# polli-labs/linnaeus

Measured on AMD Instinct MI355X. Metric: images/sec (train fwd+bwd) mFormerV1_sm 3x224x224, higher is better.
Workload: dtype bf16; 1 GPU; mFormerV1_sm train step (forward + 4-task CE loss + backward + AdamW (one HIP launch)), bf16 operands / fp32 accumulate+residual, batch 256/GPU, 3x224x224 synthetic, DropPath 0.2, gradient checkpointing off; per_gpu_batch=256, global_batch=256, parallelism=dp1, grad_mode=direct

## Files before the change

### include/lnx.h

```cpp
#ifndef LNX_H
#define LNX_H
#include <stdint.h>

#ifdef __cplusplus
extern "C" {
#endif

#define LNX_F32 0
#define LNX_BF16 1

const char* lnx_last_error(void);
int lnx_version(void);
int lnx_device_cus(void);
int lnx_set_cu_margin(int cus);
int lnx_set_deterministic(int on);
int lnx_get_deterministic(void);
int lnx_tile_sched_static(void);

typedef struct lnx_rowmap {
    int group, pad, off;
} lnx_rowmap;

enum { LNX_ACT_NONE = 0, LNX_ACT_GELU = 1, LNX_ACT_RELU = 2, LNX_ACT_GELU_BWD = 3, LNX_ACT_RELU_BWD = 4,
       LNX_ACT_GELU_D = 5, LNX_ACT_MUL_AUX = 6 };
// ... 201 lines not shown
int lnx_dwconv7_wgrad_kept(const lnx_dwconv_wgrad_args* args, const int* perm, const int* nkeep, void* stream);
int64_t lnx_dwconv7_wgrad_ws_floats(int B, int H, int W, int C, int x_dtype, int dy_dtype);

enum { LNX_ROPE_COS = 0, LNX_ROPE_ROTATE = 1 };
int lnx_rope_cos_table(const float* freqs , int heads, int H, int W, float* cos_out ,
                       float* dsin_out ,
                       void* stream);
int lnx_rope_cos_table_hd(const float* freqs, int heads, int head_dim, int H, int W, float* cos_out, float* dsin_out, void* stream);
int lnx_rope_cossin_table_hd(const float* freqs, int heads, int head_dim, int H, int W, float* cos_out, float* sin_out, float* dsin_out, void* stream);
#define LNX_ROPE_TABLES_MAX 24
typedef struct {
    const float* freqs;
    float* cos_out;
    float* dsin_out;
    int heads, H, W;
    int head_dim;
    int rope_mode;
    float* sin_out;
} lnx_rope_table;
int lnx_rope_cos_tables(const lnx_rope_table* tables, int n, void* stream);
int64_t lnx_attn_bwd_ws_floats(int B, int N, int heads);
int64_t lnx_attn_bwd_ws_floats_hd(int B, int N, int heads, int head_dim);

typedef struct lnx_attn_args {
    int dtype;
    int B, N, E, heads;
    const void* qkv;
    const float* cos_tab;
    void* o;
    float* lse;
    const unsigned char* drop_mask;
    float drop_inv_keep;
    int head_dim;
    int rope_mode;
    const float* sin_tab;
} lnx_attn_args;
int lnx_attn_fwd(const lnx_attn_args* args, void* stream);

typedef struct lnx_attn_bwd_args {
    int dtype;
    int B, N, E, heads;
    const void* qkv;
    const float* cos_tab;
    const void* o;
    const float* lse;
    const void* d_o;
    void* dqkv;
    float* freq_ws;
    float* delta;
    const unsigned char* drop_mask;
    float drop_inv_keep;
    const float* dsin_tab;
    float* dfreqs;
    int defer_freqs;
    int head_dim;
    int rope_mode;
    const float* sin_tab;
    int grid_w;
} lnx_attn_bwd_args;
#define LNX_ATTN_DEFER_MAX 16
int lnx_attn_bwd_flush(void* stream);
int lnx_attn_bwd_discard(void);
int lnx_attn_bwd(const lnx_attn_bwd_args* args, void* stream);
int lnx_attn_bwd_sized(const lnx_attn_bwd_args* args, int64_t freq_ws_floats, void* stream);
int lnx_attn_fwd_compact(const lnx_attn_args* args, const int* nkeep, void* stream);
int lnx_attn_bwd_compact(const lnx_attn_bwd_args* args, const int* nkeep, int64_t freq_ws_floats, void* stream);

enum { LNX_ATTN_KERNEL_NONE = 0, LNX_ATTN_KERNEL_RES4 = 1 , LNX_ATTN_KERNEL_RES8 = 2 ,
       LNX_ATTN_KERNEL_TILED4 = 3 , LNX_ATTN_KERNEL_TILED8 = 4  };
int lnx_attn_dispatch(int dtype, int N, int head_dim, int has_drop_mask);
int lnx_last_attn_kernel(void);
int lnx_last_attn_bwd_launches(void);

int lnx_im2col_stem(const float* x, int B, int Cin, int H, int W, void* patches, int dtype, int ldp, void* stream);

typedef struct lnx_stem_args {
    const float* x;
    const void* w;
    const float* bias;
    const float* ln_w;
    const float* ln_b;
    void* patches;
    void* pre;
    float* y;
    float* mean;
    float* rstd;
    int B, Cin, H, W, Cout;
    float eps;
} lnx_stem_args;
int lnx_stem_fwd_ok(int dtype, int Cin, int H, int W, int Cout);
int lnx_stem_fwd(const lnx_stem_args* args, void* stream);

int lnx_scale_cast(const float* in, int64_t ldin, lnx_rowmap in_map, const float* rowscale, int rows_per_sample, void* out,
                   int out_dtype, int64_t ldout, int M, int C, void* stream);

#define LNX_DROP_LIST_INTS(B) (2 * (B) + 2)
#define LNX_DROP_PARTITION_MAX 64
int lnx_drop_partition(const float* scales, int n_calls, int B, const unsigned char* call_mask, const int* rows_per_sample, int* lists, void* stream);
int lnx_scale_cast_compact(const float* in, int64_t ldin, const float* rowscale, int rows_per_sample, const int* perm, const int* m_dev, void* out,
                           int out_dtype, int64_t ldout, int M, int C, void* stream);

int lnx_copy_dropped_rows(const float* src, float* dst, int64_t ld, const int* perm, const int* nkeep, int B, int rows_per_sample, int C, void* stream);

int lnx_set_drop_compact(int on);
int64_t lnx_drop_compact_branches(void);
int64_t lnx_drop_compact_conv_blocks(void);
int lnx_set_last_cls(int on);
int64_t lnx_last_cls_blocks(void);

int lnx_layerscale_bwd(const float* g, const void* z, int dtype, const float* gamma, const float* rowscale,
                       int rows_per_sample, void* dz, float* dgamma, int M, int C, void* stream);

int lnx_layerscale_apply_wgrad(const float* s, const float* t, int64_t lds, const float* w, const float* b, int64_t ldw, const float* gamma, float* dw, float* db,
                               int64_t lddw, float* dgamma, int C, int K, void* stream);

int lnx_dropout_mul(void* x, int dtype, const unsigned char* mask, float inv_keep, int M, int C, void* stream);
int lnx_dropout_residual(const void* z, int z_dtype, const unsigned char* mask, float inv_keep, const float* rowscale, int rows_per_sample,
                         const float* res, float* out, int M, int C, void* stream);

int lnx_fill_rows(const float* vec, float* out, int64_t ldout, lnx_rowmap map, int M, int C, void* stream);
int lnx_layerscale_bwd_ws(const float* g, const void* z, int dtype, const float* gamma, const float* rowscale, int rows_per_sample, void* dz,
                          float* dgamma, int M, int C, float* ws, int64_t ws_floats, void* stream);
int64_t lnx_layerscale_bwd_ws_floats(int M, int C);
int lnx_colsum_rows(const float* in, int64_t ldin, lnx_rowmap map, float* out, int M, int C, void* stream);

int lnx_agg2_fwd(const float* a, const float* b, const float* w2, const float* bias1, float* out, int M, int C, void* stream);
int lnx_agg2_bwd(const float* dout, const float* a, const float* b, const float* w2, float* da, float* db_, float* dw2,
                 float* dbias1, int M, int C, void* stream);

int lnx_pack_meta(const float* meta, int width, int off, int dim, void* out, int dtype, int B, void* stream);

typedef struct lnx_meta_head_args {
    int B, C;
    int dim, off;
    const float* meta;
    int meta_width;
    float eps;
    const float* w0;
    int ldw0;
    const float *b0, *ln0_w, *ln0_b;
    const float* w1;
    int ldw1;
    const float *b1, *ln1_w, *ln1_b;
    const float* w2;
    int ldw2;
    const float *b2, *ln2_w, *ln2_b;
    float* t0;
    float *h0, *x, *h1, *n1, *h2;
    float *m0, *r0, *m1, *r1, *m2, *r2;
    float* tok;
    int64_t tok_row_stride, tok_row_offset;
// ... 604 lines not shown
```

### linnaeus_amd/_lib.py

```python
from __future__ import annotations

import ctypes as C
import os

_HERE = os.path.dirname(os.path.abspath(__file__))
LIB_PATH = os.environ.get("LNX_LIB_PATH") or os.path.join(_HERE, "liblnx_hip.so")

F32, BF16 = 0, 1
ACT_NONE, ACT_GELU, ACT_RELU, ACT_GELU_BWD, ACT_RELU_BWD, ACT_GELU_D, ACT_MUL_AUX = 0, 1, 2, 3, 4, 5, 6
TN_WS_FLOATS = 256 * (256 * 128 + 256)
DROP_PARTITION_MAX = 64


def drop_list_ints(B: int) -> int:
    return 2 * B + 2
ADDR_PLAIN, ADDR_PATCH2 = 0, 1


class LnxError(RuntimeError):
    pass


class RowMap(C.Structure):
    _fields_ = [("group", C.c_int), ("pad", C.c_int), ("off", C.c_int)]
# ... 320 lines not shown
        if hasattr(_lib, "lnx_hier_refine_fwd"):
            _lib.lnx_hier_refine_fwd.argtypes = [C.POINTER(HierRefineArgs), C.c_void_p]
            _lib.lnx_hier_refine_bwd.argtypes = [C.POINTER(HierRefineArgs), C.c_void_p]
            _lib.lnx_hier_refine_launches.restype = C.c_int64
        if hasattr(_lib, "lnx_abstain_act"):
            _lib.lnx_abstain_act.argtypes = [C.POINTER(AbstainActArgs), C.c_void_p]
            _lib.lnx_ppo_advantages.argtypes = [C.POINTER(PpoAdvArgs), C.c_void_p]
            _lib.lnx_ppo_loss_fwd.argtypes = [C.POINTER(PpoLossArgs), C.c_void_p]
            _lib.lnx_ppo_loss_bwd.argtypes = [C.POINTER(PpoLossArgs), C.c_void_p, C.c_void_p]
            _lib.lnx_abstain_launches.restype = C.c_int64
        if hasattr(_lib, "lnx_preprocess"):
            _lib.lnx_resize_taps.argtypes = [C.c_int, C.c_int, C.c_int]
            _lib.lnx_resize_coeffs.argtypes = [C.c_int, C.c_int, C.c_int, C.c_void_p, C.c_void_p]
            _lib.lnx_preprocess_scratch_bytes.argtypes = [C.POINTER(PreprocessImage), C.c_int, C.c_int, C.c_int, C.c_int]
            _lib.lnx_preprocess_scratch_bytes.restype = C.c_int64
            _lib.lnx_preprocess.argtypes = [C.POINTER(PreprocessArgs), C.c_void_p]
            _lib.lnx_preprocess.restype = C.c_int
        if hasattr(_lib, "lnx_meta_mask"):
            _lib.lnx_meta_mask.argtypes = [C.POINTER(MetaMaskArgs), C.c_void_p]
            _lib.lnx_meta_mask.restype = C.c_int
        if hasattr(_lib, "lnx_drop_partition"):
            _lib.lnx_drop_partition.argtypes = [C.c_void_p, C.c_int, C.c_int, C.c_char_p, C.POINTER(C.c_int), C.c_void_p, C.c_void_p]
            _lib.lnx_copy_dropped_rows.argtypes = [C.c_void_p, C.c_void_p, C.c_int64, C.c_void_p, C.c_void_p, C.c_int, C.c_int, C.c_int, C.c_void_p]
            _lib.lnx_drop_compact_branches.restype = C.c_int64
            if hasattr(_lib, "lnx_drop_compact_conv_blocks"):
                _lib.lnx_drop_compact_conv_blocks.restype = C.c_int64
                _lib.lnx_dwconv7_fwd_kept.argtypes = [C.POINTER(DwconvArgs), C.c_void_p, C.c_void_p, C.c_void_p]
                _lib.lnx_dwconv7_wgrad_kept.argtypes = [C.POINTER(DwconvWgradArgs), C.c_void_p, C.c_void_p, C.c_void_p]
            _lib.lnx_scale_cast_compact.argtypes = [C.c_void_p, C.c_int64, C.c_void_p, C.c_int, C.c_void_p, C.c_void_p, C.c_void_p, C.c_int, C.c_int64, C.c_int, C.c_int,
                                                    C.c_void_p]
        if hasattr(_lib, "lnx_last_cls_blocks"):
            _lib.lnx_set_last_cls.argtypes = [C.c_int]
            _lib.lnx_last_cls_blocks.restype = C.c_int64
        if hasattr(_lib, "lnx_plan_forward_tail"):
            _lib.lnx_plan_forward_tail.argtypes = [C.c_void_p, C.c_void_p, C.c_void_p, C.c_void_p, C.c_void_p]
            _lib.lnx_plan_trunk_valid.argtypes = [C.c_void_p]
        if hasattr(_lib, "lnx_plan_set_trainable"):
            _lib.lnx_plan_unit_name.argtypes = [C.c_void_p, C.c_int]
            _lib.lnx_plan_unit_name.restype = C.c_char_p
            _lib.lnx_plan_set_trainable.argtypes = [C.c_void_p, C.c_char_p]
        if hasattr(_lib, "lnx_gemm_tn_query"):
            _lib.lnx_gemm_tn_query.argtypes = [C.POINTER(WgradArgs), C.POINTER(TnLaunch)]
        if hasattr(_lib, "lnx_layernorm_fwd_query"):
            _lib.lnx_layernorm_fwd_query.argtypes = [C.POINTER(LnArgs), C.POINTER(LnLaunch)]
            _lib.lnx_layernorm_bwd_query.argtypes = [C.POINTER(LnBwdArgs), C.POINTER(LnLaunch)]
        older = bool(os.environ.get("LNX_LIB_PATH")) and os.environ.get("LNX_LIB_OLDER") == "1"
        for name in EXPORTS:
            if not hasattr(_lib, name) and not older:
                raise LnxError(f"{LIB_PATH} does not export {name}; rebuild it")
    return _lib


def set_deterministic(on: bool) -> bool:
    return bool(lib().lnx_set_deterministic(1 if on else 0))


def is_deterministic() -> bool:
    return bool(lib().lnx_get_deterministic())


def check(rc: int, what: str) -> None:
    if rc != 0:
        raise LnxError(f"{what} failed (rc={rc}): {lib().lnx_last_error().decode()}")


AUG_CLAMP, AUG_POSTERIZE, AUG_SOLARIZE, AUG_SOLARIZE_ADD, AUG_INVERT, AUG_BRIGHTNESS, AUG_CONTRAST = range(7)

NT_KERNEL_NONE, NT_KERNEL_V1, NT_KERNEL_V2, NT_KERNEL_SKINNY, NT_KERNEL_V4, NT_KERNEL_FP8, NT_KERNEL_V7, NT_KERNEL_MX8, NT_KERNEL_V9, NT_KERNEL_EXPERIMENT = 0, 1, 2, 3, 4, 6, 7, 8, 9, 15

ROPE_COS, ROPE_ROTATE = 0, 1

ATTN_KERNEL_NONE, ATTN_KERNEL_RES4, ATTN_KERNEL_RES8, ATTN_KERNEL_TILED4, ATTN_KERNEL_TILED8 = range(5)

EXPORTS = [
    "lnx_last_error", "lnx_version", "lnx_device_cus", "lnx_set_cu_margin", "lnx_set_deterministic", "lnx_get_deterministic", "lnx_tile_sched_static",
    "lnx_gemm_nt", "lnx_last_nt_kernel", "lnx_nt_kernel_launches", "lnx_nt_dispatch", "lnx_gemm_tn", "lnx_gemm_tn_query", "lnx_gemm_tn_flush", "lnx_gemm_tn_discard", "lnx_amax", "lnx_quantize_fp8", "lnx_gemm_nt_fp8", "lnx_quantize_mxfp8", "lnx_gemm_nt_mxfp8", "lnx_dropout_mul", "lnx_dropout_residual", "lnx_plan_dropout_bytes", "lnx_plan_set_dropout", "lnx_plan_attn_dropout_bytes", "lnx_plan_set_attn_dropout",
    "lnx_layernorm_fwd", "lnx_layernorm_bwd", "lnx_layernorm_bwd_flush", "lnx_layernorm_bwd_discard", "lnx_layernorm_fwd_query", "lnx_layernorm_bwd_query",
    "lnx_dwconv7_fwd", "lnx_dwconv7_fwd_kept", "lnx_dwconv7_wgrad", "lnx_dwconv7_wgrad_kept", "lnx_dwconv7_wgrad_ws_floats",
    "lnx_gemm_nt_group_ok", "lnx_gemm_nt_group", "lnx_rope_cos_table", "lnx_rope_cos_table_hd", "lnx_rope_cossin_table_hd", "lnx_rope_cos_tables", "lnx_attn_bwd_ws_floats", "lnx_attn_bwd_ws_floats_hd", "lnx_attn_fwd", "lnx_attn_bwd", "lnx_attn_bwd_sized", "lnx_attn_fwd_compact", "lnx_attn_bwd_compact", "lnx_attn_bwd_flush", "lnx_attn_bwd_discard", "lnx_attn_dispatch", "lnx_last_attn_kernel", "lnx_last_attn_bwd_launches",
    "lnx_im2col_stem", "lnx_scale_cast", "lnx_scale_cast_compact", "lnx_drop_partition", "lnx_copy_dropped_rows", "lnx_set_drop_compact", "lnx_drop_compact_branches", "lnx_drop_compact_conv_blocks", "lnx_set_last_cls", "lnx_last_cls_blocks", "lnx_layerscale_bwd", "lnx_layerscale_bwd_ws", "lnx_layerscale_bwd_ws_floats", "lnx_layerscale_apply_wgrad", "lnx_fill_rows", "lnx_colsum_rows",
    "lnx_agg2_fwd", "lnx_agg2_bwd", "lnx_pack_meta", "lnx_meta_heads_supported", "lnx_meta_heads_fwd", "lnx_meta_heads_bwd", "lnx_meta_heads_bwd_part_floats", "lnx_prep_weights", "lnx_prep_blocks", "lnx_softce", "lnx_softce_multi", "lnx_taxonomy_rows", "lnx_stem_fwd", "lnx_stem_fwd_ok", "lnx_adamw_blocks", "lnx_grad_sumsq", "lnx_adamw_step", "lnx_ademamix_step", "lnx_sgd_step", "lnx_optim_launches", "lnx_grad_sumsq_guarded", "lnx_adamw_step_guarded", "lnx_ademamix_step_guarded", "lnx_sgd_step_guarded", "lnx_muon_layout", "lnx_muon_step", "lnx_muon_launches", "lnx_muon_partition", "lnx_muon_orthogonalize", "lnx_muon_apply_packed", "lnx_gradnorm_sumsq", "lnx_gradnorm_update",
    "lnx_metrics_table_sizes", "lnx_metrics_update", "lnx_predict", "lnx_resize_taps", "lnx_resize_coeffs", "lnx_preprocess_scratch_bytes", "lnx_preprocess", "lnx_hier_loss_fwd", "lnx_hier_loss_bwd",
    "lnx_hier_refine_fwd", "lnx_hier_refine_bwd", "lnx_hier_refine_launches",
    "lnx_abstain_act", "lnx_ppo_advantages", "lnx_ppo_loss_fwd", "lnx_ppo_loss_bwd", "lnx_abstain_launches",
    "lnx_mix_rows", "lnx_mix_meta", "lnx_meta_mask",
    "lnx_aug_pointwise", "lnx_aug_saturation", "lnx_aug_rowstat", "lnx_aug_rescale", "lnx_aug_affine", "lnx_aug_stencil", "lnx_erase_rects", "lnx_u8hwc_to_f32chw",
    "lnx_convmlp_supported", "lnx_convmlp_fwd", "lnx_convmlp_bwd", "lnx_convmlp_bwd_ws_floats",
    "lnx_plan_create", "lnx_plan_destroy", "lnx_plan_workspace_bytes", "lnx_plan_num_params", "lnx_plan_param_name",
    "lnx_plan_param_numel", "lnx_plan_num_drop_calls", "lnx_plan_logits_numel", "lnx_plan_logits_offset", "lnx_plan_logits_ld",
    "lnx_plan_bind", "lnx_plan_forward", "lnx_plan_forward_tail", "lnx_plan_trunk_valid", "lnx_plan_backward", "lnx_plan_backward_into", "lnx_plan_segment_params", "lnx_plan_profile_begin", "lnx_plan_profile_end", "lnx_plan_profile_begin_spans", "lnx_plan_profile_end_ex", "lnx_plan_set_wgrad_stream", "lnx_plan_set_meta_stream",
    "lnx_plan_num_units", "lnx_plan_unit_name", "lnx_plan_param_unit", "lnx_plan_set_trainable", "lnx_plan_first_trained_unit", "lnx_plan_last_backward_units",
]


class MetaHeadArgs(C.Structure):
    _fields_ = [
        ("B", C.c_int), ("C", C.c_int), ("dim", C.c_int), ("off", C.c_int),
        ("meta", C.c_void_p), ("meta_width", C.c_int), ("eps", C.c_float),
        ("w0", C.c_void_p), ("ldw0", C.c_int), ("b0", C.c_void_p), ("ln0_w", C.c_void_p), ("ln0_b", C.c_void_p),
        ("w1", C.c_void_p), ("ldw1", C.c_int), ("b1", C.c_void_p), ("ln1_w", C.c_void_p), ("ln1_b", C.c_void_p),
        ("w2", C.c_void_p), ("ldw2", C.c_int), ("b2", C.c_void_p), ("ln2_w", C.c_void_p), ("ln2_b", C.c_void_p),
        ("t0", C.c_void_p), ("h0", C.c_void_p), ("x", C.c_void_p), ("h1", C.c_void_p), ("n1", C.c_void_p), ("h2", C.c_void_p),
        ("m0", C.c_void_p), ("r0", C.c_void_p), ("m1", C.c_void_p), ("r1", C.c_void_p), ("m2", C.c_void_p), ("r2", C.c_void_p),
        ("tok", C.c_void_p), ("tok_row_stride", C.c_int64), ("tok_row_offset", C.c_int64),
    ]


class MetaHeadBwdArgs(C.Structure):
    _fields_ = [
        ("B", C.c_int), ("C", C.c_int), ("dim", C.c_int),
        ("g", C.c_void_p), ("g_row_stride", C.c_int64), ("g_row_offset", C.c_int64),
        ("w1t", C.c_void_p), ("ldw1t", C.c_int), ("w2t", C.c_void_p), ("ldw2t", C.c_int),
        ("ln0_w", C.c_void_p), ("ln1_w", C.c_void_p), ("ln2_w", C.c_void_p),
# ... 42 lines not shown
class LnLaunch(C.Structure):
    _fields_ = [("G", C.c_int), ("V", C.c_int), ("pair", C.c_int), ("full", C.c_int), ("mx", C.c_int), ("grid", C.c_int), ("cols", C.c_int), ("slices", C.c_int)]


class RopeTable(C.Structure):
    _fields_ = [
        ("freqs", C.c_void_p), ("cos_out", C.c_void_p), ("dsin_out", C.c_void_p),
        ("heads", C.c_int), ("H", C.c_int), ("W", C.c_int), ("head_dim", C.c_int),
        ("rope_mode", C.c_int), ("sin_out", C.c_void_p),
    ]


class DwconvArgs(C.Structure):
    _fields_ = [
        ("B", C.c_int), ("H", C.c_int), ("W", C.c_int), ("C", C.c_int),
        ("x", C.c_void_p), ("x_dtype", C.c_int), ("w49", C.c_void_p), ("bias", C.c_void_p),
        ("flip", C.c_int), ("res", C.c_void_p), ("y", C.c_void_p), ("y_dtype", C.c_int),
    ]


class DwconvWgradArgs(C.Structure):
    _fields_ = [
        ("B", C.c_int), ("H", C.c_int), ("W", C.c_int), ("C", C.c_int),
        ("x", C.c_void_p), ("x_dtype", C.c_int), ("dy", C.c_void_p), ("dy_dtype", C.c_int),
        ("dw", C.c_void_p), ("db", C.c_void_p),
        ("ws", C.c_void_p), ("ws_floats", C.c_int64),
    ]


class AttnArgs(C.Structure):
    _fields_ = [
        ("dtype", C.c_int), ("B", C.c_int), ("N", C.c_int), ("E", C.c_int), ("heads", C.c_int),
        ("qkv", C.c_void_p), ("cos_tab", C.c_void_p), ("o", C.c_void_p), ("lse", C.c_void_p),
        ("drop_mask", C.c_void_p), ("drop_inv_keep", C.c_float), ("head_dim", C.c_int),
        ("rope_mode", C.c_int), ("sin_tab", C.c_void_p),
    ]


class AttnBwdArgs(C.Structure):
    _fields_ = [
        ("dtype", C.c_int), ("B", C.c_int), ("N", C.c_int), ("E", C.c_int), ("heads", C.c_int),
        ("qkv", C.c_void_p), ("cos_tab", C.c_void_p), ("o", C.c_void_p), ("lse", C.c_void_p),
        ("d_o", C.c_void_p), ("dqkv", C.c_void_p), ("freq_ws", C.c_void_p), ("delta", C.c_void_p),
        ("drop_mask", C.c_void_p), ("drop_inv_keep", C.c_float),
        ("dsin_tab", C.c_void_p), ("dfreqs", C.c_void_p), ("defer_freqs", C.c_int), ("head_dim", C.c_int),
        ("rope_mode", C.c_int), ("sin_tab", C.c_void_p), ("grid_w", C.c_int),
    ]


class PrepDesc(C.Structure):
    _fields_ = [
        ("src", C.c_void_p), ("dst", C.c_void_p), ("dst_t", C.c_void_p),
        ("rows", C.c_int), ("cols", C.c_int), ("ld", C.c_int), ("ld_t", C.c_int),
        ("P", C.c_int), ("mode", C.c_int), ("block_start", C.c_int),
    ]


PREP_CAST, PREP_CONV_PERM, PREP_DW49 = 0, 1, 2


class ConvMlpArgs(C.Structure):
    _fields_ = [
        ("dtype", C.c_int), ("M", C.c_int), ("C", C.c_int),
        ("ln", C.c_void_p), ("w1", C.c_void_p), ("b1", C.c_void_p), ("w2", C.c_void_p), ("b2", C.c_void_p),
        ("gamma", C.c_void_p), ("rowscale", C.c_void_p), ("rows_per_sample", C.c_int),
        ("x", C.c_void_p), ("out", C.c_void_p), ("z", C.c_void_p),
        ("y", C.c_void_p), ("ln_w", C.c_void_p), ("ln_b", C.c_void_p), ("ln_eps", C.c_float), ("ln_out", C.c_void_p),
        ("mean", C.c_void_p), ("rstd", C.c_void_p),
        ("perm", C.c_void_p), ("m_dev", C.c_void_p),
    ]


class ConvMlpBwdArgs(C.Structure):
    _fields_ = [
        ("dtype", C.c_int), ("M", C.c_int), ("C", C.c_int),
        ("g", C.c_void_p), ("ln", C.c_void_p), ("z", C.c_void_p), ("w1", C.c_void_p), ("b1", C.c_void_p),
        ("w2t", C.c_void_p), ("w1t", C.c_void_p), ("gamma", C.c_void_p), ("rowscale", C.c_void_p), ("rows_per_sample", C.c_int),
        ("act", C.c_void_p), ("dh", C.c_void_p), ("dz", C.c_void_p), ("dln", C.c_void_p), ("dgamma", C.c_void_p),
# ... 33 lines not shown
```

### linnaeus_amd/csrc/api.cpp

```cpp
#include <hip/hip_runtime.h>
#include <stdarg.h>
#include <stdio.h>
#include <stdlib.h>
#include <string.h>

#include <atomic>
#include <mutex>

#include "../../include/lnx.h"

static thread_local char g_err[1024] = "";

void lnx_set_error(const char* fmt, ...) {
    va_list ap;
    va_start(ap, fmt);
    vsnprintf(g_err, sizeof(g_err), fmt, ap);
    va_end(ap);
}

extern "C" const char* lnx_last_error(void) { return g_err; }
extern "C" int lnx_version(void) { return 120; }
extern "C" int lnx_device_cus(void) {
    int dev = 0;
    if (hipGetDevice(&dev) != hipSuccess) return -1;
    hipDeviceProp_t prop;
    if (hipGetDeviceProperties(&prop, dev) != hipSuccess) return -1;
    return prop.multiProcessorCount;
}

static std::atomic<int> g_cu_margin{-1};
int persistent_cus(int cus) {
    int m = g_cu_margin.load(std::memory_order_relaxed);
    if (m < 0) {
        const char* e = getenv("LNX_CU_MARGIN");
        m = e ? atoi(e) : 0;
        if (m < 0) m = 0;
        g_cu_margin.store(m, std::memory_order_relaxed);
    }
    const int room = cus - m;
    return room < 8 ? 8 : room;
}
void set_cu_margin(int m) { g_cu_margin.store(m < 0 ? 0 : m, std::memory_order_relaxed); }
static std::atomic<int> g_deterministic{-1};
bool deterministic() {
    int d = g_deterministic.load(std::memory_order_relaxed);
    if (d < 0) {
        const char* e = getenv("LNX_DETERMINISTIC");
        d = e && atoi(e) == 1 ? 1 : 0;
        int unset = -1;
        if (!g_deterministic.compare_exchange_strong(unset, d, std::memory_order_relaxed)) d = unset;
    }
    return d != 0;
}
extern "C" int lnx_get_deterministic(void) { return deterministic() ? 1 : 0; }
// ... 42 lines not shown
```

### linnaeus_amd/csrc/attention.hip

```cpp
#include <stdlib.h>

#include <atomic>
#include <vector>

#include "common.hpp"
#include "../../include/lnx.h"

namespace {

constexpr int BT = 64;

typedef __attribute__((ext_vector_type(4))) short s16x4_t;

template <typename T, int HD = 64> struct AT {
    static_assert(HD == 32 || HD == 64 || HD == 128, "head_dim 32, 64 or 128");
    static constexpr int EPV = TT<T>::EPV;
    static constexpr int NKK = HD * (int)sizeof(T) / 64;
    static constexpr int ND = HD / 16;
    static constexpr int ROWB = HD * sizeof(T);
    static constexpr int NCH = ROWB / 16;
    static constexpr int SWZ = (NCH < 8 ? NCH : 8) - 1;
    static constexpr int TRB = ROWB + (sizeof(T) == 2 ? 32 : 16);
    static constexpr int ROW_IMG = BT * ROWB;
    static constexpr int TR_IMG = BT * TRB;
// ... 305 lines not shown
    static __device__ __forceinline__ float prep(float m) {
        if constexpr (sizeof(T) == 2) return m * L2E;
        else return m;
    }
    static __device__ __forceinline__ float sub(float x, float mp) {
        if constexpr (sizeof(T) == 2) return __builtin_amdgcn_exp2f(fmaf(x, L2E, -mp));
        else return expf(x - mp);
    }
    static __device__ __forceinline__ float clamped(float x, float mp) {
        if constexpr (sizeof(T) == 2) return __builtin_amdgcn_exp2f(fminf(fmaf(x, L2E, -mp), 0.f));
        else return expf(fminf(x - mp, 0.f));
    }
};

struct AttnP {
    const void* qkv;
    const float* cos_tab;
    void* o;
    float* lse;
    const void* d_o;
    void* dqkv;
    float* fpart;
    const float* dsin;
    float* delta;
    int B, N, E, heads;
    int qtiles;
    const unsigned char* amask = nullptr;
    float a_inv_keep = 1.0f;
    int Np = 0;
    const float* sin_tab = nullptr;
    int W = 1;
    float* fwave = nullptr;
    const int* nkeep = nullptr;
};

template <int HD = 64> __device__ __forceinline__ float* freq_wave_slot(const AttnP& p) {
    if (p.fwave == nullptr) return nullptr;
    const int wave = __builtin_amdgcn_readfirstlane(threadIdx.x >> 6), lane = threadIdx.x & 63;
    float* fw = p.fwave + ((int64_t)blockIdx.x * FREQ_WAVES + wave) * HD;
    if ((lane & 15) == 0) {
#pragma unroll
        for (int dt = 0; dt < HD / 16; ++dt)
#pragma unroll
            for (int pr = 0; pr < 2; ++pr) {
                const int j = 8 * dt + 2 * (lane >> 4) + pr;
                fw[j] = 0.f;
                fw[HD / 2 + j] = 0.f;
            }
    }
    return fw;
}

template <typename T, int HD = 64, bool ROT = false>
__device__ __forceinline__ void dkv_epilogue(const AttnP& p, const f32x4_t (&dk)[HD / 16], const f32x4_t (&dv)[HD / 16], const T* __restrict__ kb, int64_t ld, int C,
                                             int b, int head, int key, int s, int g, float* fl, float* fw) {
    const int kc = min(key, p.N - 1);
    const T* kraw = kb + (int64_t)kc * ld;
    const float* cpr = p.cos_tab + ((int64_t)max(kc - p.E, 0) * p.heads + head) * (HD / 2);
    const float* sxp = p.dsin + ((int64_t)max(kc - p.E, 0) * p.heads + head) * (HD / 2);
    const float* syp = sxp + (int64_t)(p.N - p.E) * p.heads * (HD / 2);
    constexpr int ND = HD / 16;
    float kr[ND][4], cr[ND][2], gp[ND][2], dx[ND][2], dy[ND][2];
    float sr[ROT ? ND : 1][2];
    const bool rope = p.E < p.N;
#pragma unroll
    for (int dt = 0; dt < ND; ++dt) {
// ... 34 lines not shown
        float ok[ND][4];
#pragma unroll
        for (int dt = 0; dt < ND; ++dt) {
            const float c0 = img ? cr[dt][0] : 1.0f, c1 = img ? cr[dt][1] : 1.0f;
            if constexpr (ROT) {
                const float s0 = img ? sr[dt][0] : 0.f, s1 = img ? sr[dt][1] : 0.f;
                ok[dt][0] = dk[dt][0] * c0 + dk[dt][1] * s0; ok[dt][1] = dk[dt][1] * c0 - dk[dt][0] * s0;
                ok[dt][2] = dk[dt][2] * c1 + dk[dt][3] * s1; ok[dt][3] = dk[dt][3] * c1 - dk[dt][2] * s1;
                const float x0 = kr[dt][0] * c0 - kr[dt][1] * s0, x1 = kr[dt][0] * s0 + kr[dt][1] * c0;
                const float x2 = kr[dt][2] * c1 - kr[dt][3] * s1, x3 = kr[dt][2] * s1 + kr[dt][3] * c1;
                gp[dt][0] = img ? dk[dt][1] * x0 - dk[dt][0] * x1 : 0.f;
                gp[dt][1] = img ? dk[dt][3] * x2 - dk[dt][2] * x3 : 0.f;
                continue;
            }
            ok[dt][0] = dk[dt][0] * c0; ok[dt][1] = dk[dt][1] * c0; ok[dt][2] = dk[dt][2] * c1; ok[dt][3] = dk[dt][3] * c1;
            gp[dt][0] = img ? dk[dt][0] * kr[dt][0] + dk[dt][1] * kr[dt][1] : 0.f;
            gp[dt][1] = img ? dk[dt][2] * kr[dt][2] + dk[dt][3] * kr[dt][3] : 0.f;
        }
        store_row<T, HD>(dkp, ok, g, row);
    }
    {
        float ov[ND][4];
#pragma unroll
        for (int dt = 0; dt < ND; ++dt)
#pragma unroll
            for (int j = 0; j < 4; ++j) ov[dt][j] = dv[dt][j];
        store_row<T, HD>(dkp + C, ov, g, row);
    }
    if (rope) freq_accum<HD>(fl, fw, gp, dx, dy, s, g);
}
template <typename T, int HD = 64, bool ROT = false>
__device__ __forceinline__ void dq_epilogue(const AttnP& p, const f32x4_t (&dq)[HD / 16], const T* __restrict__ qb, int64_t ld, int b, int head, int q, int s, int g,
                                            float scale, float* fl, float* fw) {
    const int qc = min(q, p.N - 1);
    const T* qraw = qb + (int64_t)qc * ld;
    const float* cpr = p.cos_tab + ((int64_t)max(qc - p.E, 0) * p.heads + head) * (HD / 2);
    const float* sxp = p.dsin + ((int64_t)max(qc - p.E, 0) * p.heads + head) * (HD / 2);
    const float* syp = sxp + (int64_t)(p.N - p.E) * p.heads * (HD / 2);
    constexpr int ND = HD / 16;
    float qr[ND][4], cr[ND][2], gp[ND][2], dx[ND][2], dy[ND][2];
    float sr[ROT ? ND : 1][2];
    const bool rope = p.E < p.N;
#pragma unroll
    for (int dt = 0; dt < ND; ++dt) {
        const int d0 = dt * 16 + 4 * g;
        if constexpr (sizeof(T) == 2) {
            const uint2 r = *reinterpret_cast<const uint2*>(qraw + d0);
            const bf16_t* h = reinterpret_cast<const bf16_t*>(&r);
#pragma unroll
            for (int j = 0; j < 4; ++j) qr[dt][j] = (float)h[j];
        } else {
            const float4 r = *reinterpret_cast<const float4*>(qraw + d0);
            qr[dt][0] = r.x; qr[dt][1] = r.y; qr[dt][2] = r.z; qr[dt][3] = r.w;
        }
        cr[dt][0] = cr[dt][1] = 1.0f;
        dx[dt][0] = dx[dt][1] = dy[dt][0] = dy[dt][1] = 0.f;
        if constexpr (ROT) {
            sr[dt][0] = sr[dt][1] = 0.f;
            if (rope) {
                const float2 c2 = *reinterpret_cast<const float2*>(cpr + (d0 >> 1));
                const float2 s2 = *reinterpret_cast<const float2*>(p.sin_tab + ((int64_t)max(qc - p.E, 0) * p.heads + head) * (HD / 2) + (d0 >> 1));
                cr[dt][0] = c2.x; cr[dt][1] = c2.y;
                sr[dt][0] = s2.x; sr[dt][1] = s2.y;
                dx[dt][0] = dx[dt][1] = (float)(max(qc - p.E, 0) % p.W);
                dy[dt][0] = dy[dt][1] = (float)(max(qc - p.E, 0) / p.W);
            }
        } else if (rope) {
            const float2 c2 = *reinterpret_cast<const float2*>(cpr + (d0 >> 1));
            cr[dt][0] = c2.x; cr[dt][1] = c2.y;
            const float2 a2 = *reinterpret_cast<const float2*>(sxp + (d0 >> 1));
            const float2 b2 = *reinterpret_cast<const float2*>(syp + (d0 >> 1));
            dx[dt][0] = a2.x; dx[dt][1] = a2.y;
            dy[dt][0] = b2.x; dy[dt][1] = b2.y;
        }
    }
    const bool row = q < p.N, img = row && q >= p.E;
    T* dqp = reinterpret_cast<T*>(p.dqkv) + ((int64_t)b * p.N + qc) * ld + head * HD;
    float oq[ND][4];
#pragma unroll
    for (int dt = 0; dt < ND; ++dt) {
        if constexpr (ROT) {
            const float s0 = img ? sr[dt][0] : 0.f, s1 = img ? sr[dt][1] : 0.f, r0 = img ? cr[dt][0] : 1.0f, r1 = img ? cr[dt][1] : 1.0f;
            oq[dt][0] = scale * (dq[dt][0] * r0 + dq[dt][1] * s0); oq[dt][1] = scale * (dq[dt][1] * r0 - dq[dt][0] * s0);
            oq[dt][2] = scale * (dq[dt][2] * r1 + dq[dt][3] * s1); oq[dt][3] = scale * (dq[dt][3] * r1 - dq[dt][2] * s1);
            const float x0 = qr[dt][0] * r0 - qr[dt][1] * s0, x1 = qr[dt][0] * s0 + qr[dt][1] * r0;
            const float x2 = qr[dt][2] * r1 - qr[dt][3] * s1, x3 = qr[dt][2] * s1 + qr[dt][3] * r1;
            gp[dt][0] = img ? scale * (dq[dt][1] * x0 - dq[dt][0] * x1) : 0.f;
            gp[dt][1] = img ? scale * (dq[dt][3] * x2 - dq[dt][2] * x3) : 0.f;
            continue;
        }
        const float c0 = img ? cr[dt][0] * scale : scale, c1 = img ? cr[dt][1] * scale : scale;
        oq[dt][0] = dq[dt][0] * c0; oq[dt][1] = dq[dt][1] * c0; oq[dt][2] = dq[dt][2] * c1; oq[dt][3] = dq[dt][3] * c1;
        gp[dt][0] = img ? scale * (dq[dt][0] * qr[dt][0] + dq[dt][1] * qr[dt][1]) : 0.f;
        gp[dt][1] = img ? scale * (dq[dt][2] * qr[dt][2] + dq[dt][3] * qr[dt][3]) : 0.f;
    }
    store_row<T, HD>(dqp, oq, g, row);
    if (rope) freq_accum<HD>(fl, fw, gp, dx, dy, s, g);
}

template <typename T, int NW = 4, bool DROP = false, int HD = 64, bool ROT = false>
__global__ __launch_bounds__(64 * NW) void attn_fwd_kernel(const AttnP p) {
    extern __shared__ __attribute__((aligned(16))) unsigned char smem[];
    unsigned char* kimg = smem;
    unsigned char* vimg = smem + AT<T, HD>::ROW_IMG;
    const int lane = threadIdx.x & 63, wave = threadIdx.x >> 6;
    const int s = lane & 15, g = lane >> 4;
    const int qt = blockIdx.x % p.qtiles;
    const int bh = blockIdx.x / p.qtiles;
    const int head = bh % p.heads, b = bh / p.heads;
    if (p.nkeep && b >= *p.nkeep) return;
    const int C = p.heads * HD;
    const int64_t ld = 3 * C;
    const T* qb = reinterpret_cast<const T*>(p.qkv) + (int64_t)b * p.N * ld + head * HD;
    const T* kb = qb + C;
    const T* vb = qb + 2 * C;
    const float scale = attn_scale<HD>();

    const int q = qt * (16 * NW) + wave * 16 + s;
    uint4 qf[(AT<T, HD>::NKK)];
    load_row_frag<T, true, HD, ROT>(qf, qb, ld, q, p.N, p.E, g, p.cos_tab, p.heads, head, scale, p.sin_tab);

    f32x4_t oacc[HD / 16];
#pragma unroll
    for (int i = 0; i < HD / 16; ++i) oacc[i] = f32x4_t{0.f, 0.f, 0.f, 0.f};
    float m_run = -INFINITY, l_run = 0.f;
    const unsigned char* mrow = nullptr;
    if constexpr (DROP) mrow = p.amask + (((int64_t)b * p.heads + head) * p.N + min(q, p.N - 1)) * p.Np + 4 * g;

    const int nkt = (p.N + BT - 1) / BT;
    TileFetch<T, true, 64 * NW, HD, ROT> fk;
    TileFetch<T, false, 64 * NW, HD> fv;
    fk.fetch(kb, ld, 0, p.N, p.E, p.cos_tab, p.heads, head, p.sin_tab);
    fv.fetch(vb, ld, 0, p.N, p.E, nullptr, p.heads, head);
    for (int kt = 0; kt < nkt; ++kt) {
        uint32_t mk[4] = {0, 0, 0, 0};
        if constexpr (DROP) {
#pragma unroll
            for (int t = 0; t < 4; ++t) mk[t] = *reinterpret_cast<const uint32_t*>(mrow + kt * BT + 16 * t);
        }
        __syncthreads();
        fk.template commit<true, false>(kimg, nullptr, kt * BT, p.N, p.E, 1.0f);
        fv.template commit<false, true>(nullptr, vimg, kt * BT, p.N, p.E, 1.0f);
        const int nxt = min(kt + 1, nkt - 1) * BT;
        fk.fetch(kb, ld, nxt, p.N, p.E, p.cos_tab, p.heads, head, p.sin_tab);
        fv.fetch(vb, ld, nxt, p.N, p.E, nullptr, p.heads, head);
        __syncthreads();
        f32x4_t sacc[4];
        rows_times_frag_n<T, 4, HD>(sacc, kimg, s, g, qf);
        float pv[4][4];
        float mx = -INFINITY;
        if (kt * BT + BT <= p.N) {
#pragma unroll
            for (int t = 0; t < 4; ++t)
// ... 12 lines not shown
                    pv[t][r] = v;
                    mx = fmaxf(mx, v);
                }
        }
        mx = group_max(mx);
        const float m_new = fmaxf(m_run, mx);
        const float mp = RowExp<T>::prep(m_new);
        const float alpha = RowExp<T>::sub(m_run, mp);
        float psum = 0.f;
#pragma unroll
        for (int t = 0; t < 4; ++t)
#pragma unroll
            for (int r = 0; r < 4; ++r) {
                const float e = RowExp<T>::sub(pv[t][r], mp);
                psum += e;
                pv[t][r] = DROP ? (((mk[t] >> (8 * r)) & 0xffu) ? e * p.a_inv_keep : 0.f) : e;
            }
        l_run = l_run * alpha + psum;
        m_run = m_new;
#pragma unroll
        for (int dt = 0; dt < HD / 16; ++dt)
#pragma unroll
            for (int r = 0; r < 4; ++r) oacc[dt][r] *= alpha;
        imgT_times_regs_n<T, 4, HD>(oacc, vimg, s, g, pv);
    }
    const float l_tot = group_sum(l_run);
    const float inv = 1.0f / l_tot;
    {
        float ov[HD / 16][4];
#pragma unroll
        for (int dt = 0; dt < HD / 16; ++dt)
#pragma unroll
            for (int r = 0; r < 4; ++r) ov[dt][r] = oacc[dt][r] * inv;
        store_row<T, HD>(reinterpret_cast<T*>(p.o) + ((int64_t)b * p.N + min(q, p.N - 1)) * C + head * HD, ov, g, q < p.N);
        if (q < p.N && g == 0 && p.lse) p.lse[((int64_t)b * p.heads + head) * p.N + q] = m_run + logf(l_tot);
    }
}

template <typename T, int NW = 4, bool DROP = false, int HD = 64, bool ROT = false>
__global__ __launch_bounds__(64 * NW) void attn_bwd_dq_kernel(const AttnP p) {
    extern __shared__ __attribute__((aligned(16))) unsigned char smem[];
    unsigned char* kimg = smem;
    unsigned char* vimg = smem + AT<T, HD>::ROW_IMG;
    unsigned char* ktr = smem + 2 * AT<T, HD>::ROW_IMG;
    const int lane = threadIdx.x & 63, wave = threadIdx.x >> 6;
    const int s = lane & 15, g = lane >> 4;
    const int qt = blockIdx.x % p.qtiles;
    const int bh = blockIdx.x / p.qtiles;
    const int head = bh % p.heads, b = bh / p.heads;
    if (p.nkeep && b >= *p.nkeep) return;
    const int C = p.heads * HD;
    const int64_t ld = 3 * C;
    const T* qb = reinterpret_cast<const T*>(p.qkv) + (int64_t)b * p.N * ld + head * HD;
    const T* kb = qb + C;
    const T* vb = qb + 2 * C;
    const T* dob = reinterpret_cast<const T*>(p.d_o) + (int64_t)b * p.N * C + head * HD;
    const T* ob = reinterpret_cast<const T*>(p.o) + (int64_t)b * p.N * C + head * HD;
    const float scale = attn_scale<HD>();

    __shared__ float fl[HD];
    float* fw = freq_wave_slot<HD>(p);
    if (threadIdx.x < HD) fl[threadIdx.x] = 0.f;
    const int q = qt * (16 * NW) + wave * 16 + s;
    uint4 qf[(AT<T, HD>::NKK)], dof[(AT<T, HD>::NKK)];
    load_row_frag<T, true, HD, ROT>(qf, qb, ld, q, p.N, p.E, g, p.cos_tab, p.heads, head, scale, p.sin_tab);
    load_row_frag<T, false, HD>(dof, dob, C, q, p.N, p.E, g, nullptr, p.heads, head, 1.0f);
    float dl = 0.f;
    {
        uint4 of[(AT<T, HD>::NKK)];
        load_row_frag<T, false, HD>(of, ob, C, q, p.N, p.E, g, nullptr, p.heads, head, 1.0f);
#pragma unroll
        for (int kk = 0; kk < AT<T, HD>::NKK; ++kk) {
            Vec16<T> a, bb;
            a.raw = dof[kk];
            bb.raw = of[kk];
#pragma unroll
            for (int j = 0; j < AT<T, HD>::EPV; ++j) dl += a.get(j) * bb.get(j);
        }
    }
    const float delta = group_sum(dl);
    const float lse_raw = p.lse[((int64_t)b * p.heads + head) * p.N + min(q, p.N - 1)];
    const float lse = RowExp<T>::prep(q < p.N ? lse_raw : 0.f);
    if (q < p.N && g == 0) p.delta[((int64_t)b * p.heads + head) * p.N + q] = delta;

    f32x4_t dq[HD / 16];
#pragma unroll
    for (int i = 0; i < HD / 16; ++i) dq[i] = f32x4_t{0.f, 0.f, 0.f, 0.f};
    const unsigned char* mrow = nullptr;
    if constexpr (DROP) mrow = p.amask + (((int64_t)b * p.heads + head) * p.N + min(q, p.N - 1)) * p.Np + 4 * g;

    const int nkt = (p.N + BT - 1) / BT;
    TileFetch<T, true, 64 * NW, HD, ROT> fk;
    TileFetch<T, false, 64 * NW, HD> fv;
    fk.fetch(kb, ld, 0, p.N, p.E, p.cos_tab, p.heads, head, p.sin_tab);
    fv.fetch(vb, ld, 0, p.N, p.E, nullptr, p.heads, head);
    for (int kt = 0; kt < nkt; ++kt) {
        uint32_t mk[4] = {0, 0, 0, 0};
        if constexpr (DROP) {
#pragma unroll
            for (int t = 0; t < 4; ++t) mk[t] = *reinterpret_cast<const uint32_t*>(mrow + kt * BT + 16 * t);
        }
        __syncthreads();
        fk.template commit<true, true>(kimg, ktr, kt * BT, p.N, p.E, 1.0f);
        fv.template commit<true, false>(vimg, nullptr, kt * BT, p.N, p.E, 1.0f);
        const int nxt = min(kt + 1, nkt - 1) * BT;
        fk.fetch(kb, ld, nxt, p.N, p.E, p.cos_tab, p.heads, head, p.sin_tab);
        fv.fetch(vb, ld, nxt, p.N, p.E, nullptr, p.heads, head);
        __syncthreads();
#pragma unroll
        for (int h = 0; h < 2; ++h) {
            f32x4_t sacc[4], dpacc[4];
            rows_times_frag_n<T, 2, HD>(sacc, kimg + h * 32 * AT<T, HD>::ROWB, s, g, qf);
            PHASE_FENCE();
            rows_times_frag_n<T, 2, HD>(dpacc, vimg + h * 32 * AT<T, HD>::ROWB, s, g, dof);
            PHASE_FENCE();
            float ds[4][4];
// ... 26 lines not shown
    unsigned char* qtr = smem + 2 * AT<T, HD>::ROW_IMG;
    unsigned char* dotr = qtr + AT<T, HD>::TR_IMG;
    float* lse_s = reinterpret_cast<float*>(dotr + AT<T, HD>::TR_IMG);
    float* del_s = lse_s + BT;
    const int lane = threadIdx.x & 63, wave = threadIdx.x >> 6;
    const int s = lane & 15, g = lane >> 4;
    const int ktile = blockIdx.x % p.qtiles;
    const int bh = blockIdx.x / p.qtiles;
    const int head = bh % p.heads, b = bh / p.heads;
    if (p.nkeep && b >= *p.nkeep) return;
    const int C = p.heads * HD;
    const int64_t ld = 3 * C;
    const T* qb = reinterpret_cast<const T*>(p.qkv) + (int64_t)b * p.N * ld + head * HD;
    const T* kb = qb + C;
    const T* vb = qb + 2 * C;
    const T* dob = reinterpret_cast<const T*>(p.d_o) + (int64_t)b * p.N * C + head * HD;
    const float scale = attn_scale<HD>();
    const int64_t statbase = ((int64_t)b * p.heads + head) * p.N;

    __shared__ float fl[HD];
    float* fw = freq_wave_slot<HD>(p);
    if (threadIdx.x < HD) fl[threadIdx.x] = 0.f;
    const int key = ktile * (16 * NW) + wave * 16 + s;
    uint4 kf[(AT<T, HD>::NKK)], vf[(AT<T, HD>::NKK)];
    load_row_frag<T, true, HD, ROT>(kf, kb, ld, key, p.N, p.E, g, p.cos_tab, p.heads, head, 1.0f, p.sin_tab);
    load_row_frag<T, false, HD>(vf, vb, ld, key, p.N, p.E, g, nullptr, p.heads, head, 1.0f);

    f32x4_t dk[HD / 16], dv[HD / 16];
#pragma unroll
    for (int i = 0; i < HD / 16; ++i) {
        dk[i] = f32x4_t{0.f, 0.f, 0.f, 0.f};
        dv[i] = f32x4_t{0.f, 0.f, 0.f, 0.f};
    }
    const int nqt = (p.N + BT - 1) / BT;
    TileFetch<T, true, 64 * NW, HD, ROT> fq;
    TileFetch<T, false, 64 * NW, HD> fdo;
    const int stl = threadIdx.x & (BT - 1);
    float l_n, d_n;
    fq.fetch(qb, ld, 0, p.N, p.E, p.cos_tab, p.heads, head, p.sin_tab);
    fdo.fetch(dob, C, 0, p.N, p.E, nullptr, p.heads, head);
    l_n = p.lse[statbase + min(stl, p.N - 1)];
    d_n = p.delta[statbase + min(stl, p.N - 1)];
    for (int qt = 0; qt < nqt; ++qt) {
        __syncthreads();
        fq.template commit<true, true>(qimg, qtr, qt * BT, p.N, p.E, scale);
        fdo.template commit<true, true>(doimg, dotr, qt * BT, p.N, p.E, 1.0f);
        if (threadIdx.x < BT) {
            const int qq = qt * BT + threadIdx.x;
            lse_s[threadIdx.x] = RowExp<T>::prep(qq < p.N ? l_n : 0.f);
            del_s[threadIdx.x] = qq < p.N ? d_n : 0.f;
        }
        const int nxt = min(qt + 1, nqt - 1) * BT;
        fq.fetch(qb, ld, nxt, p.N, p.E, p.cos_tab, p.heads, head, p.sin_tab);
        fdo.fetch(dob, C, nxt, p.N, p.E, nullptr, p.heads, head);
        l_n = p.lse[statbase + min(nxt + stl, p.N - 1)];
        d_n = p.delta[statbase + min(nxt + stl, p.N - 1)];
        __syncthreads();
#pragma unroll
        for (int h = 0; h < 2; ++h) {
            f32x4_t sacc[4], dpacc[4];
            rows_times_frag_n<T, 2, HD>(sacc, qimg + h * 32 * AT<T, HD>::ROWB, s, g, kf);
            PHASE_FENCE();
            rows_times_frag_n<T, 2, HD>(dpacc, doimg + h * 32 * AT<T, HD>::ROWB, s, g, vf);
            PHASE_FENCE();
            float pr[4][4], ds[4][4];
#pragma unroll
            for (int t = 0; t < 4; ++t) {
                if (t < 2) {
                    const float4 l4 = *reinterpret_cast<const float4*>(lse_s + h * 32 + t * 16 + 4 * g);
                    const float4 d4 = *reinterpret_cast<const float4*>(del_s + h * 32 + t * 16 + 4 * g);
                    const float lv[4] = {l4.x, l4.y, l4.z, l4.w}, dvv[4] = {d4.x, d4.y, d4.z, d4.w};
#pragma unroll
                    for (int r = 0; r < 4; ++r) {
                        const float pp = RowExp<T>::clamped(sacc[t][r], lv[r]);
                        float keepf = 1.0f;
                        if constexpr (DROP) {
                            const int qq = qt * BT + h * 32 + t * 16 + 4 * g + r;
                            keepf = p.amask[(((int64_t)b * p.heads + head) * p.N + min(qq, p.N - 1)) * p.Np + min(key, p.N - 1)] ? p.a_inv_keep : 0.f;
                        }
                        pr[t][r] = pp * keepf;
                        ds[t][r] = pp * (dpacc[t][r] * keepf - dvv[r]);
                    }
                } else {
#pragma unroll
                    for (int r = 0; r < 4; ++r) pr[t][r] = ds[t][r] = 0.f;
                }
            }
            PHASE_FENCE();
            imgT_times_regs_n<T, 2, HD>(dv, dotr + h * 32 * AT<T, HD>::TRB, s, g, pr);
// ... 35 lines not shown
template <typename T, bool COS, bool ROWIMG, bool TRIMG, bool ROT = false>
__device__ __forceinline__ void stage_all(unsigned char* rowimg, unsigned char* trimg, const T* __restrict__ base, int64_t ld, int nrows_pad, int N, int E,
                                          const float* __restrict__ cos_tab, int heads, int head, float scale, const float* __restrict__ sin_tab = nullptr) {
    constexpr int UN = 4;
    const int total = nrows_pad * AT<T>::NCH;
    for (int i0 = threadIdx.x; i0 < total; i0 += UN * blockDim.x) {
        StageBatch<T, COS, ROT, UN> sb;
        sb.fetch(base, ld, i0, total, N, E, cos_tab, heads, head, sin_tab);
        sb.template commit<ROWIMG, TRIMG>(rowimg, trimg, i0, total, N, E, scale);
    }
}

template <typename T, int NW = 8, bool ROT = false>
__global__ __launch_bounds__(64 * NW) __attribute__((amdgpu_waves_per_eu(4, 4))) void attn_fwd_res_kernel(const AttnP p) {
    extern __shared__ __attribute__((aligned(16))) unsigned char smem[];
    constexpr int HD = 64;
    const int nkt = (p.N + BT - 1) / BT;
    const int npad = nkt * BT;
    unsigned char* kimg = smem;
    unsigned char* vimg = smem + npad * AT<T>::ROWB;
    const int lane = threadIdx.x & 63, wave = threadIdx.x >> 6;
    const int s = lane & 15, g = lane >> 4;
    const int head = blockIdx.x % p.heads, b = blockIdx.x / p.heads;
    if (p.nkeep && b >= *p.nkeep) return;
    const int C = p.heads * HD;
    const int64_t ld = 3 * C;
    const T* qb = reinterpret_cast<const T*>(p.qkv) + (int64_t)b * p.N * ld + head * HD;
    const T* kb = qb + C;
    const T* vb = qb + 2 * C;
    const float scale = 0.125f;
    stage_all<T, true, true, false, ROT>(kimg, nullptr, kb, ld, npad, p.N, p.E, p.cos_tab, p.heads, head, 1.0f, p.sin_tab);
    stage_all<T, false, false, true>(nullptr, vimg, vb, ld, npad, p.N, p.E, nullptr, p.heads, head, 1.0f);
    __syncthreads();
    const int nq16 = (p.N + 15) / 16;
    for (int qt = wave; qt < nq16; qt += NW) {
        const int q = qt * 16 + s;
        uint4 qf[AT<T>::NKK];
        load_row_frag<T, true, 64, ROT>(qf, qb, ld, q, p.N, p.E, g, p.cos_tab, p.heads, head, scale, p.sin_tab);
        f32x4_t oacc[4];
#pragma unroll
        for (int i = 0; i < 4; ++i) oacc[i] = f32x4_t{0.f, 0.f, 0.f, 0.f};
        float m_run = -INFINITY, l_run = 0.f;
        auto kstep = [&](const int kt, auto ntc, auto maskc) __attribute__((always_inline)) {
            constexpr int NT = decltype(ntc)::value;
            constexpr bool MASK = decltype(maskc)::value != 0;
            f32x4_t sacc[4];
            rows_times_frag_n<T, NT>(sacc, kimg + kt * BT * AT<T>::ROWB, s, g, qf);
            float pv[4][4];
            float mx = -INFINITY;
#pragma unroll
            for (int t = 0; t < NT; ++t)
#pragma unroll
                for (int r = 0; r < 4; ++r) {
                    float v = sacc[t][r];
                    if constexpr (MASK) v = kt * BT + t * 16 + 4 * g + r < p.N ? v : -INFINITY;
                    pv[t][r] = v;
                    mx = fmaxf(mx, v);
                }
            mx = group_max(mx);
            const float m_new = fmaxf(m_run, mx);
            const float mp = RowExp<T>::prep(m_new);
            const float alpha = RowExp<T>::sub(m_run, mp);
            float psum = 0.f;
#pragma unroll
            for (int t = 0; t < 4; ++t)
#pragma unroll
                for (int r = 0; r < 4; ++r) {
                    const float e = t < NT ? RowExp<T>::sub(pv[t][r], mp) : 0.f;
                    pv[t][r] = e;
                    psum += e;
                }
            l_run = l_run * alpha + psum;
            m_run = m_new;
#pragma unroll
            for (int dt = 0; dt < 4; ++dt)
#pragma unroll
                for (int r = 0; r < 4; ++r) oacc[dt][r] *= alpha;
            imgT_times_regs_n<T, NT>(oacc, vimg + kt * BT * AT<T>::TRB, s, g, pv);
        };
        const int nf = p.N / BT;
        for (int kt = 0; kt < nf; ++kt) kstep(kt, IC<4>{}, IC<0>{});
        if (nf < nkt) {
            if (p.N - nf * BT > 32) kstep(nf, IC<4>{}, IC<1>{});
            else kstep(nf, IC<2>{}, IC<1>{});
        }
        const float l_tot = group_sum(l_run);
        const float inv = 1.0f / l_tot;
        {
            float ov[4][4];
#pragma unroll
            for (int dt = 0; dt < 4; ++dt)
#pragma unroll
                for (int r = 0; r < 4; ++r) ov[dt][r] = oacc[dt][r] * inv;
            store_row<T>(reinterpret_cast<T*>(p.o) + ((int64_t)b * p.N + min(q, p.N - 1)) * C + head * HD, ov, g, q < p.N);
            if (q < p.N && g == 0 && p.lse) p.lse[((int64_t)b * p.heads + head) * p.N + q] = m_run + logf(l_tot);
        }
    }
}

template <typename T, bool ROT>
__device__ __forceinline__ void dq_res_prefetch(float (&qr)[4][4], float (&cr)[4][2], const AttnP& p, const T* __restrict__ qb, int64_t ld, int qc, int head, int g) {
    const T* qraw = qb + (int64_t)qc * ld;
    const float* cpr = p.cos_tab + ((int64_t)max(qc - p.E, 0) * p.heads + head) * 32;
#pragma unroll
    for (int dt = 0; dt < 4; ++dt) {
        const int d0 = dt * 16 + 4 * g;
        if constexpr (sizeof(T) == 2) {
            const uint2 r = *reinterpret_cast<const uint2*>(qraw + d0);
            const bf16_t* h = reinterpret_cast<const bf16_t*>(&r);
#pragma unroll
            for (int j = 0; j < 4; ++j) qr[dt][j] = (float)h[j];
        } else {
            const float4 r = *reinterpret_cast<const float4*>(qraw + d0);
            qr[dt][0] = r.x; qr[dt][1] = r.y; qr[dt][2] = r.z; qr[dt][3] = r.w;
        }
        if constexpr (!ROT) {
            const float2 c2 = *reinterpret_cast<const float2*>(cpr + (d0 >> 1));
            cr[dt][0] = c2.x; cr[dt][1] = c2.y;
        }
    }
}
template <typename T>
__device__ __forceinline__ void dq_res_loop(f32x4_t (&dq)[4], const unsigned char* kimg, const unsigned char* vimg, int npad, int s, int g,
                                            const uint4 (&qf)[AT<T>::NKK], const uint4 (&dof)[AT<T>::NKK], float lse, float delta) {
    for (int k0 = 0; k0 < npad; k0 += 32) {
        f32x4_t sacc[4], dpacc[4];
        rows_times_frag_pad_n<T, 2>(sacc, kimg + k0 * AT<T>::TRB, s, g, qf);
        PHASE_FENCE();
        rows_times_frag_pad_n<T, 2>(dpacc, vimg + k0 * AT<T>::TRB, s, g, dof);
        PHASE_FENCE();
        float ds[4][4];
#pragma unroll
        for (int t = 0; t < 4; ++t)
#pragma unroll
            for (int r = 0; r < 4; ++r) ds[t][r] = t < 2 ? RowExp<T>::clamped(sacc[t][r], lse) * (dpacc[t][r] - delta) : 0.f;
        PHASE_FENCE();
        imgT_times_regs_n<T, 2>(dq, kimg + k0 * AT<T>::TRB, s, g, ds);
        PHASE_FENCE();
    }
}
template <typename T, bool ROT>
__device__ __forceinline__ void dq_res_epilogue(const AttnP& p, const f32x4_t (&dq)[4], const float (&qr)[4][4], float (&cr)[4][2], int64_t ld, int b, int head, int q,
                                                int s, int g, float scale, float* fl, float* fw) {
    constexpr int HD = 64;
    const int qc = min(q, p.N - 1);
    const float* cpr = p.cos_tab + ((int64_t)max(qc - p.E, 0) * p.heads + head) * 32;
    const float* sxp = p.dsin + ((int64_t)max(qc - p.E, 0) * p.heads + head) * 32;
    const float* syp = sxp + (int64_t)(p.N - p.E) * p.heads * 32;
    float gp[4][2], dx[4][2], dy[4][2];
    float sr[ROT ? 4 : 1][2];
#pragma unroll
    for (int dt = 0; dt < 4; ++dt) {
        if constexpr (ROT) {
            const float2 c2 = *reinterpret_cast<const float2*>(cpr + ((dt * 16 + 4 * g) >> 1));
            const float2 s2 = *reinterpret_cast<const float2*>(p.sin_tab + ((int64_t)max(qc - p.E, 0) * p.heads + head) * 32 + ((dt * 16 + 4 * g) >> 1));
            cr[dt][0] = c2.x; cr[dt][1] = c2.y;
            sr[dt][0] = s2.x; sr[dt][1] = s2.y;
            dx[dt][0] = dx[dt][1] = (float)(max(qc - p.E, 0) % p.W);
            dy[dt][0] = dy[dt][1] = (float)(max(qc - p.E, 0) / p.W);
            continue;
        }
        const float2 a = *reinterpret_cast<const float2*>(sxp + ((dt * 16 + 4 * g) >> 1));
        const float2 c = *reinterpret_cast<const float2*>(syp + ((dt * 16 + 4 * g) >> 1));
        dx[dt][0] = a.x; dx[dt][1] = a.y;
        dy[dt][0] = c.x; dy[dt][1] = c.y;
    }
    const bool row = q < p.N, img = row && q >= p.E;
    T* dqp = reinterpret_cast<T*>(p.dqkv) + ((int64_t)b * p.N + qc) * ld + head * HD;
    float oq[4][4];
#pragma unroll
    for (int dt = 0; dt < 4; ++dt) {
        if constexpr (ROT) {
            const float s0 = img ? sr[dt][0] : 0.f, s1 = img ? sr[dt][1] : 0.f, r0 = img ? cr[dt][0] : 1.0f, r1 = img ? cr[dt][1] : 1.0f;
            oq[dt][0] = scale * (dq[dt][0] * r0 + dq[dt][1] * s0); oq[dt][1] = scale * (dq[dt][1] * r0 - dq[dt][0] * s0);
            oq[dt][2] = scale * (dq[dt][2] * r1 + dq[dt][3] * s1); oq[dt][3] = scale * (dq[dt][3] * r1 - dq[dt][2] * s1);
            const float x0 = qr[dt][0] * r0 - qr[dt][1] * s0, x1 = qr[dt][0] * s0 + qr[dt][1] * r0;
            const float x2 = qr[dt][2] * r1 - qr[dt][3] * s1, x3 = qr[dt][2] * s1 + qr[dt][3] * r1;
            gp[dt][0] = img ? scale * (dq[dt][1] * x0 - dq[dt][0] * x1) : 0.f;
            gp[dt][1] = img ? scale * (dq[dt][3] * x2 - dq[dt][2] * x3) : 0.f;
            continue;
        }
        const float c0 = img ? cr[dt][0] * scale : scale, c1 = img ? cr[dt][1] * scale : scale;
        oq[dt][0] = dq[dt][0] * c0; oq[dt][1] = dq[dt][1] * c0; oq[dt][2] = dq[dt][2] * c1; oq[dt][3] = dq[dt][3] * c1;
        gp[dt][0] = img ? scale * (dq[dt][0] * qr[dt][0] + dq[dt][1] * qr[dt][1]) : 0.f;
        gp[dt][1] = img ? scale * (dq[dt][2] * qr[dt][2] + dq[dt][3] * qr[dt][3]) : 0.f;
    }
    store_row<T>(dqp, oq, g, row);
    if (p.E < p.N) freq_accum(fl, fw, gp, dx, dy, s, g);
}
template <typename T>
__device__ __forceinline__ float delta_of_row(const uint4 (&dof)[AT<T>::NKK], const uint4 (&of)[AT<T>::NKK]) {
    float dl = 0.f;
#pragma unroll
    for (int kk = 0; kk < AT<T>::NKK; ++kk) {
        Vec16<T> a, bb;
        a.raw = dof[kk];
        bb.raw = of[kk];
#pragma unroll
        for (int j = 0; j < AT<T>::EPV; ++j) dl += a.get(j) * bb.get(j);
    }
// ... 30 lines not shown
        imgT_times_regs_n<T, 2>(dv, doimg + q0 * AT<T>::TRB, s, g, pr);
        PHASE_FENCE();
        imgT_times_regs_n<T, 2>(dk, qimg + q0 * AT<T>::TRB, s, g, ds);
        PHASE_FENCE();
    }
}

template <typename T, int NW = 8, bool ROT = false>
__global__ __launch_bounds__(64 * NW) __attribute__((amdgpu_waves_per_eu(4, 4))) void attn_bwd_dq_res_kernel(const AttnP p) {
    extern __shared__ __attribute__((aligned(16))) unsigned char smem[];
    constexpr int HD = 64;
    const int nkt = (p.N + BT - 1) / BT;
    const int npad = (p.N + 31) & ~31;
    unsigned char* kimg = smem;
    unsigned char* vimg = kimg + npad * AT<T>::TRB;
    const int lane = threadIdx.x & 63, wave = threadIdx.x >> 6;
    const int s = lane & 15, g = lane >> 4;
    const int head = blockIdx.x % p.heads, b = blockIdx.x / p.heads;
    if (p.nkeep && b >= *p.nkeep) return;
    const int C = p.heads * HD;
    const int64_t ld = 3 * C;
    const T* qb = reinterpret_cast<const T*>(p.qkv) + (int64_t)b * p.N * ld + head * HD;
    const T* kb = qb + C;
    const T* vb = qb + 2 * C;
    const T* dob = reinterpret_cast<const T*>(p.d_o) + (int64_t)b * p.N * C + head * HD;
    const T* ob = reinterpret_cast<const T*>(p.o) + (int64_t)b * p.N * C + head * HD;
    const float scale = 0.125f;
    __shared__ float fl[64];
    float* fw = freq_wave_slot<64>(p);
    if (threadIdx.x < 64) fl[threadIdx.x] = 0.f;
    stage_all<T, true, false, true, ROT>(nullptr, kimg, kb, ld, npad, p.N, p.E, p.cos_tab, p.heads, head, 1.0f, p.sin_tab);
    stage_all<T, false, false, true>(nullptr, vimg, vb, ld, npad, p.N, p.E, nullptr, p.heads, head, 1.0f);
    __syncthreads();
    const int nq16 = (p.N + 15) / 16;
    for (int qt = wave; qt < nq16; qt += NW) {
        const int q = qt * 16 + s;
        const int qc = min(q, p.N - 1);
        uint4 qf[AT<T>::NKK], dof[AT<T>::NKK];
        Chunk<T, true, 64, ROT> cq[AT<T>::NKK];
        Chunk<T, false> cdo[AT<T>::NKK], co[AT<T>::NKK];
#pragma unroll
        for (int kk = 0; kk < AT<T>::NKK; ++kk) {
            const int d0 = (kk * 4 + g) * AT<T>::EPV;
            cq[kk].fetch(qb, ld, q, p.N, p.E, d0, p.cos_tab, p.heads, head, p.sin_tab);
            cdo[kk].fetch(dob, C, q, p.N, p.E, d0, nullptr, p.heads, head);
            co[kk].fetch(ob, C, q, p.N, p.E, d0, nullptr, p.heads, head);
        }
        const float lse_raw = p.lse[((int64_t)b * p.heads + head) * p.N + qc];
        float qr[4][4], cr[4][2];
        dq_res_prefetch<T, ROT>(qr, cr, p, qb, ld, qc, head, g);
#pragma unroll
        for (int kk = 0; kk < AT<T>::NKK; ++kk) {
            qf[kk] = cq[kk].value(q, p.N, p.E, scale);
            dof[kk] = cdo[kk].value(q, p.N, p.E, 1.0f);
        }
        uint4 of[AT<T>::NKK];
#pragma unroll
        for (int kk = 0; kk < AT<T>::NKK; ++kk) of[kk] = co[kk].value(q, p.N, p.E, 1.0f);
        const float delta = delta_of_row<T>(dof, of);
        const float lse = RowExp<T>::prep(q < p.N ? lse_raw : 0.f);
        if (q < p.N && g == 0) p.delta[((int64_t)b * p.heads + head) * p.N + q] = delta;
        f32x4_t dq[4];
#pragma unroll
        for (int i = 0; i < 4; ++i) dq[i] = f32x4_t{0.f, 0.f, 0.f, 0.f};
        dq_res_loop<T>(dq, kimg, vimg, npad, s, g, qf, dof, lse, delta);
        dq_res_epilogue<T, ROT>(p, dq, qr, cr, ld, b, head, q, s, g, scale, fl, fw);
    }
    if (p.E < p.N) freq_flush<false>(fl, p.fpart, p.fwave);
}

#ifdef ATT_STAMP
__device__ unsigned long long g_att_stamp[8];
#define ATT_T(i) do { __builtin_amdgcn_sched_barrier(0); unsigned long long t_; asm volatile("s_memtime %0\n\ts_waitcnt lgkmcnt(0)" : "=s"(t_) :: "memory"); \
                      __builtin_amdgcn_sched_barrier(0); tsum[i] += t_ - tlast; tlast = t_; } while (0)
#else
#define ATT_T(i) do { } while (0)
#endif

template <typename T, int NW = 8, bool ROT = false>
__global__ __launch_bounds__(64 * NW) __attribute__((amdgpu_waves_per_eu(4, 4))) void attn_bwd_dkv_res_kernel(const AttnP p) {
    extern __shared__ __attribute__((aligned(16))) unsigned char smem[];
    constexpr int HD = 64;
#ifdef ATT_STAMP
    unsigned long long tsum[8] = {0, 0, 0, 0, 0, 0, 0, 0}, tlast;
    asm volatile("s_memtime %0\n\ts_waitcnt lgkmcnt(0)" : "=s"(tlast)::"memory");
#endif
    const int nqt = (p.N + BT - 1) / BT;
    const int npad = (p.N + 31) & ~31;
    unsigned char* qimg = smem;
    unsigned char* doimg = qimg + npad * AT<T>::TRB;
    float* lse_s = reinterpret_cast<float*>(doimg + npad * AT<T>::TRB);
    float* del_s = lse_s + nqt * BT;
    const int lane = threadIdx.x & 63, wave = threadIdx.x >> 6;
    const int s = lane & 15, g = lane >> 4;
    const int head = blockIdx.x % p.heads, b = blockIdx.x / p.heads;
    if (p.nkeep && b >= *p.nkeep) return;
    const int C = p.heads * HD;
    const int64_t ld = 3 * C;
    const T* qb = reinterpret_cast<const T*>(p.qkv) + (int64_t)b * p.N * ld + head * HD;
    const T* kb = qb + C;
    const T* vb = qb + 2 * C;
    const T* dob = reinterpret_cast<const T*>(p.d_o) + (int64_t)b * p.N * C + head * HD;
    const float scale = 0.125f;
    const int64_t statbase = ((int64_t)b * p.heads + head) * p.N;
    __shared__ float fl[64];
    float* fw = freq_wave_slot<64>(p);
    if (threadIdx.x < 64) fl[threadIdx.x] = 0.f;
    stage_all<T, true, false, true, ROT>(nullptr, qimg, qb, ld, npad, p.N, p.E, p.cos_tab, p.heads, head, scale, p.sin_tab);
    stage_all<T, false, false, true>(nullptr, doimg, dob, C, npad, p.N, p.E, nullptr, p.heads, head, 1.0f);
    ATT_T(0);
    for (int i = threadIdx.x; i < nqt * BT; i += blockDim.x) {
        const float l = p.lse[statbase + min(i, p.N - 1)], d = p.delta[statbase + min(i, p.N - 1)];
        lse_s[i] = RowExp<T>::prep(i < p.N ? l : 0.f);
        del_s[i] = i < p.N ? d : 0.f;
    }
    __syncthreads();
    ATT_T(1);
    const int nk16 = (p.N + 15) / 16;
    for (int ktile = wave; ktile < nk16; ktile += NW) {
        const int key = ktile * 16 + s;
        const int kc = min(key, p.N - 1);
        uint4 kf[AT<T>::NKK], vf[AT<T>::NKK];
        Chunk<T, true, 64, ROT> ck[AT<T>::NKK];
        Chunk<T, false> cv[AT<T>::NKK];
#pragma unroll
        for (int kk = 0; kk < AT<T>::NKK; ++kk) {
            const int d0 = (kk * 4 + g) * AT<T>::EPV;
            ck[kk].fetch(kb, ld, key, p.N, p.E, d0, p.cos_tab, p.heads, head, p.sin_tab);
            cv[kk].fetch(vb, ld, key, p.N, p.E, d0, nullptr, p.heads, head);
        }
#pragma unroll
        for (int kk = 0; kk < AT<T>::NKK; ++kk) {
            kf[kk] = ck[kk].value(key, p.N, p.E, 1.0f);
            vf[kk] = cv[kk].value(key, p.N, p.E, 1.0f);
        }
        f32x4_t dk[4], dv[4];
#pragma unroll
        for (int i = 0; i < 4; ++i) {
            dk[i] = f32x4_t{0.f, 0.f, 0.f, 0.f};
            dv[i] = f32x4_t{0.f, 0.f, 0.f, 0.f};
        }
        ATT_T(2);
        dkv_res_loop<T>(dk, dv, qimg, doimg, lse_s, del_s, npad, s, g, kf, vf);
        ATT_T(3);
        dkv_epilogue<T, 64, ROT>(p, dk, dv, kb, ld, C, b, head, key, s, g, fl, fw);
        ATT_T(4);
    }
    if (p.E < p.N) freq_flush<true>(fl, p.fpart, p.fwave);
#ifdef ATT_STAMP
    if (blockIdx.x == gridDim.x / 2 && threadIdx.x == 0)
        for (int i = 0; i < 8; ++i) g_att_stamp[i] = tsum[i];
#endif
}
#ifdef ATT_STAMP
extern "C" int lnx_dbg_attn_stamps(unsigned long long* out8) { return (int)hipMemcpyFromSymbol(out8, HIP_SYMBOL(g_att_stamp), 64); }
#endif

template <typename T> constexpr size_t res_bwd_fused_lds(int npad, int qtiles) { return (size_t)npad * (4 * AT<T>::TRB) + (size_t)qtiles * BT * 2 * sizeof(float); }

template <typename T, int NW = 16, bool ROT = false>
__global__ __launch_bounds__(64 * NW) __attribute__((amdgpu_waves_per_eu(4, 4))) void attn_bwd_res_kernel(const AttnP p) {
    extern __shared__ __attribute__((aligned(16))) unsigned char smem[];
    constexpr int HD = 64;
#ifdef ATT_STAMP
    unsigned long long tsum[8] = {0, 0, 0, 0, 0, 0, 0, 0}, tlast;
    asm volatile("s_memtime %0\n\ts_waitcnt lgkmcnt(0)" : "=s"(tlast)::"memory");
#endif
    constexpr int UN = 2;
    const int nqt = (p.N + BT - 1) / BT;
    const int npad = (p.N + 31) & ~31;
    unsigned char* qimg = smem;
    unsigned char* kimg = qimg + npad * AT<T>::TRB;
    unsigned char* vimg = kimg + npad * AT<T>::TRB;
    unsigned char* doimg = vimg + npad * AT<T>::TRB;
    float* lse_s = reinterpret_cast<float*>(doimg + npad * AT<T>::TRB);
    float* del_s = lse_s + nqt * BT;
    const int lane = threadIdx.x & 63, wave = threadIdx.x >> 6;
    const int s = lane & 15, g = lane >> 4;
    const int head = blockIdx.x % p.heads, b = blockIdx.x / p.heads;
    if (p.nkeep && b >= *p.nkeep) return;
    const int C = p.heads * HD;
    const int64_t ld = 3 * C;
    const T* qb = reinterpret_cast<const T*>(p.qkv) + (int64_t)b * p.N * ld + head * HD;
    const T* kb = qb + C;
    const T* vb = qb + 2 * C;
    const T* dob = reinterpret_cast<const T*>(p.d_o) + (int64_t)b * p.N * C + head * HD;
    const T* ob = reinterpret_cast<const T*>(p.o) + (int64_t)b * p.N * C + head * HD;
    const float scale = 0.125f;
    const int64_t statbase = ((int64_t)b * p.heads + head) * p.N;
    __shared__ float fl[64];
    float* fw = freq_wave_slot<64>(p);
    if (threadIdx.x < 64) fl[threadIdx.x] = 0.f;
    const int row = wave * 16 + s;
    const int ntiles = (p.N + 15) / 16;
    const bool tile = wave < ntiles;
    Chunk<T, false> co[AT<T>::NKK];
    {
        const int total = npad * AT<T>::NCH, i0 = threadIdx.x;
        StageBatch<T, true, ROT, UN> sq, sk;
        StageBatch<T, false, false, UN> sv, sdo;
        sq.fetch(qb, ld, i0, total, p.N, p.E, p.cos_tab, p.heads, head, p.sin_tab);
        sk.fetch(kb, ld, i0, total, p.N, p.E, p.cos_tab, p.heads, head, p.sin_tab);
        sv.fetch(vb, ld, i0, total, p.N, p.E, nullptr, p.heads, head);
        sdo.fetch(dob, C, i0, total, p.N, p.E, nullptr, p.heads, head);
        const float l = p.lse[statbase + min(i0, p.N - 1)];
#pragma unroll
        for (int kk = 0; kk < AT<T>::NKK; ++kk) co[kk].fetch(ob, C, row, p.N, p.E, (kk * 4 + g) * AT<T>::EPV, nullptr, p.heads, head);
        sq.template commit<false, true>(nullptr, qimg, i0, total, p.N, p.E, scale);
        sk.template commit<false, true>(nullptr, kimg, i0, total, p.N, p.E, 1.0f);
        sv.template commit<false, true>(nullptr, vimg, i0, total, p.N, p.E, 1.0f);
        sdo.template commit<false, true>(nullptr, doimg, i0, total, p.N, p.E, 1.0f);
        if (i0 < nqt * BT) {
            lse_s[i0] = RowExp<T>::prep(i0 < p.N ? l : 0.f);
            del_s[i0] = 0.f;
        }
    }
    ATT_T(0);
    __syncthreads();
    ATT_T(1);
    uint4 qf[AT<T>::NKK], dof[AT<T>::NKK];
    float delta = 0.f;
    if (tile) {
        uint4 of[AT<T>::NKK];
#pragma unroll
        for (int kk = 0; kk < AT<T>::NKK; ++kk) {
            qf[kk] = ld16(qimg + row * AT<T>::TRB + ((kk * 4 + g) << 4));
            dof[kk] = ld16(doimg + row * AT<T>::TRB + ((kk * 4 + g) << 4));
            of[kk] = co[kk].value(row, p.N, p.E, 1.0f);
        }
        delta = delta_of_row<T>(dof, of);
        if (row < p.N && g == 0) {
            p.delta[statbase + row] = delta;
            del_s[row] = delta;
        }
    }
    ATT_T(2);
    __syncthreads();
    ATT_T(3);
    if (tile) {
        const int q = row, qc = min(q, p.N - 1);
        float qr[4][4], cr[4][2];
        dq_res_prefetch<T, ROT>(qr, cr, p, qb, ld, qc, head, g);
        const float lse = lse_s[q];
        f32x4_t dq[4];
#pragma unroll
        for (int i = 0; i < 4; ++i) dq[i] = f32x4_t{0.f, 0.f, 0.f, 0.f};
        dq_res_loop<T>(dq, kimg, vimg, npad, s, g, qf, dof, lse, delta);
        ATT_T(4);
        dq_res_epilogue<T, ROT>(p, dq, qr, cr, ld, b, head, q, s, g, scale, fl, fw);
        ATT_T(5);
    }
    const int ktile = (wave + NW - ntiles % 4) % NW;
    if (ktile < ntiles) {
        const int key = ktile * 16 + s;
        uint4 kf[AT<T>::NKK], vf[AT<T>::NKK];
#pragma unroll
        for (int kk = 0; kk < AT<T>::NKK; ++kk) {
            kf[kk] = ld16(kimg + key * AT<T>::TRB + ((kk * 4 + g) << 4));
            vf[kk] = ld16(vimg + key * AT<T>::TRB + ((kk * 4 + g) << 4));
        }
        f32x4_t dk[4], dv[4];
#pragma unroll
        for (int i = 0; i < 4; ++i) {
            dk[i] = f32x4_t{0.f, 0.f, 0.f, 0.f};
            dv[i] = f32x4_t{0.f, 0.f, 0.f, 0.f};
        }
        dkv_res_loop<T>(dk, dv, qimg, doimg, lse_s, del_s, npad, s, g, kf, vf);
        ATT_T(6);
        dkv_epilogue<T, 64, ROT>(p, dk, dv, kb, ld, C, b, head, key, s, g, fl, fw);
        ATT_T(7);
    }
    if (p.E < p.N) freq_flush<false>(fl, p.fpart, p.fwave);
#ifdef ATT_STAMP
    if (blockIdx.x == gridDim.x / 2 && threadIdx.x == 0)
        for (int i = 0; i < 8; ++i) g_att_stamp[i] = tsum[i];
#endif
}

template <int HD = 64>
__device__ __forceinline__ void rope_cos_entry(const float* __restrict__ freqs, int heads, int H, int W, float* __restrict__ out, float* __restrict__ dsin, int i,
                                               float* __restrict__ sin_out = nullptr) {
    constexpr int HH = HD / 2, SH = HD == 32 ? 4 : HD == 64 ? 5 : 6;
    const int total = H * W * heads * HH;
    if (i >= total) return;
    const int j = i & (HH - 1);
    const int h = (i >> SH) % heads;
    const int n = (i >> SH) / heads;
    const float tx = (float)(n % W), ty = (float)(n / W);
    const float ax = __fmul_rn(tx, freqs[h * HH + j]);
    const float ay = __fmul_rn(ty, freqs[(heads + h) * HH + j]);
    const float th = __fadd_rn(ax, ay);
    out[i] = cosf(th);
    if (sin_out) sin_out[i] = sinf(th);
    if (dsin) {
        const float ms = -sinf(th);
        dsin[i] = tx * ms;
        dsin[total + i] = ty * ms;
    }
}

// ... 99 lines not shown

template <auto Kernel>
int attn_launch(int grid, int block, size_t lds, size_t lds_max, hipStream_t st, const AttnP& p) {
    static const hipError_t raise_dynamic_lds_limit = hipFuncSetAttribute(reinterpret_cast<const void*>(Kernel), hipFuncAttributeMaxDynamicSharedMemorySize, (int)lds_max);
    LNX_HIP(raise_dynamic_lds_limit);
    hipLaunchKernelGGL(Kernel, dim3(grid), dim3(block), lds, st, p);
    return 0;
}

bool hd_ok(int hd) { return hd == 32 || hd == 64 || hd == 128; }

const float* cos_or_stub(const float* tab, const void* qkv) { return tab ? tab : reinterpret_cast<const float*>(qkv); }

int check_attn(int dtype, int B, int N, int E, int heads, int hd, const char* who) {
    LNX_CHECK(dtype == LNX_F32 || dtype == LNX_BF16, "%s: bad dtype %d", who, dtype);
    LNX_CHECK(B > 0 && N > 0 && heads > 0 && E >= 0 && E <= N, "%s: bad shape B=%d N=%d E=%d heads=%d", who, B, N, E, heads);
    LNX_CHECK(hd_ok(hd), "%s: head_dim %d is not supported (32, 64 or 128)", who, hd);
    return 0;
}

static bool tiled_nw8(int N) {
    static const bool force4 = getenv("LNX_ATTN_NW") != nullptr && atoi(getenv("LNX_ATTN_NW")) == 4;
    return !force4 && N > 128;
}

template <typename T, int HD> constexpr bool hd_nw8() { return sizeof(T) == 2 && HD > 32; }

int attn_family(int dtype, int N, int hd, bool drop) {
    if (dtype != LNX_BF16 || drop || hd == 32) return LNX_ATTN_KERNEL_TILED4;
    if (hd == 64 && N <= 256 && getenv("LNX_ATTN_TILED") == nullptr) return N <= 64 ? LNX_ATTN_KERNEL_RES4 : LNX_ATTN_KERNEL_RES8;
    return tiled_nw8(N) ? LNX_ATTN_KERNEL_TILED8 : LNX_ATTN_KERNEL_TILED4;
}
bool is_resident(int family) { return family == LNX_ATTN_KERNEL_RES4 || family == LNX_ATTN_KERNEL_RES8; }

std::atomic<int> g_last_attn{LNX_ATTN_KERNEL_NONE};

template <typename T, int HD, class F>
int tiled_variant(AttnP& p, int family, F&& f) {
    if (p.amask) return f(IC<4>{}, IC<1>{});
    if constexpr (hd_nw8<T, HD>()) {
        if (family == LNX_ATTN_KERNEL_TILED8) {
            p.qtiles = cdiv(p.N, 128);
            return f(IC<8>{}, IC<0>{});
        }
    }
    return f(IC<4>{}, IC<0>{});
}

template <typename T, int HD, bool ROT>
int attn_fwd_tiled(AttnP& p, int family, hipStream_t st) {
    return tiled_variant<T, HD>(p, family, [&](auto nwc, auto dropc) {
        constexpr int NW = decltype(nwc)::value;
        constexpr bool DROP = decltype(dropc)::value != 0;
        constexpr size_t lds = AT<T, HD>::FWD_LDS;
        return attn_launch<attn_fwd_kernel<T, NW, DROP, HD, ROT>>(p.B * p.heads * p.qtiles, 64 * NW, lds, lds, st, p);
    });
}

template <typename T, int HD, bool ROT>
int attn_bwd_tiled(AttnP& p, int family, hipStream_t st, int& per_bh) {
    return tiled_variant<T, HD>(p, family, [&](auto nwc, auto dropc) {
        constexpr int NW = decltype(nwc)::value;
        constexpr bool DROP = decltype(dropc)::value != 0;
        constexpr size_t lds_q = AT<T, HD>::BWD_DQ_LDS, lds_k = AT<T, HD>::BWD_DKV_LDS;
        const int grid = p.B * p.heads * p.qtiles;
        per_bh = p.qtiles;
        if (int rc = attn_launch<attn_bwd_dq_kernel<T, NW, DROP, HD, ROT>>(grid, 64 * NW, lds_q, lds_q, st, p)) return rc;
        return attn_launch<attn_bwd_dkv_kernel<T, NW, DROP, HD, ROT>>(grid, 64 * NW, lds_k, lds_k, st, p);
    });
}

template <class F>
int res_variant(int family, F&& f) {
    return family == LNX_ATTN_KERNEL_RES4 ? f(IC<4>{}, 64) : f(IC<8>{}, 256);
}

template <bool ROT>
int attn_fwd_res(AttnP& p, int family, hipStream_t st) {
    typedef bf16_t T;
    return res_variant(family, [&](auto nwc, int nmax) {
        constexpr int NW = decltype(nwc)::value;
        return attn_launch<attn_fwd_res_kernel<T, NW, ROT>>(p.B * p.heads, 64 * NW, res_fwd_lds<T>(p.qtiles * BT), res_fwd_lds<T>(nmax), st, p);
    });
}

constexpr int RES_BWD_FUSED_NMAX = 224;
std::atomic<int> g_last_bwd_launches{0};
// ... 12 lines not shown
    return res_variant(family, [&](auto nwc, int nmax) {
        constexpr int NW = decltype(nwc)::value;
        if (int rc = attn_launch<attn_bwd_dq_res_kernel<T, NW, ROT>>(bh, 64 * NW, res_bwd_dq_lds<T>(npad), res_bwd_dq_lds<T>(nmax), st, p)) return rc;
        return attn_launch<attn_bwd_dkv_res_kernel<T, NW, ROT>>(bh, 64 * NW, res_bwd_dkv_lds<T>(npad, p.qtiles), res_bwd_dkv_lds<T>(nmax, nmax / BT), st, p);
    });
}

int rope_table_hd(const float* freqs, int heads, int hd, int H, int W, float* cos_out, float* dsin_out, hipStream_t st, const char* who, float* sin_out = nullptr) {
    LNX_CHECK(freqs && cos_out && heads > 0 && H > 0 && W > 0, "%s: bad arguments", who);
    LNX_CHECK(hd_ok(hd), "%s: head_dim %d is not supported (32, 64 or 128)", who, hd);
    const int total = H * W * heads * (hd / 2);
    with_hd(hd, [&](auto hdc) {
        hipLaunchKernelGGL(rope_cos_kernel<decltype(hdc)::value>, dim3(cdiv(total, 256)), dim3(256), 0, st, freqs, heads, H, W, cos_out, dsin_out, sin_out);
    });
    LNX_LAUNCH_CHECK();
    return 0;
}

template <bool ROT, class Args>
int attn_setup(const Args* a, const int* nkeep, int hd, const char* who, AttnP& p, int& family) {
    if (a->drop_mask) {
        LNX_CHECK(a->drop_inv_keep >= 1.0f && (((uintptr_t)a->drop_mask) & 3) == 0, "%s: drop_inv_keep >= 1 and a 4-byte aligned mask", who);
    }
    p.qkv = a->qkv; p.cos_tab = cos_or_stub(a->cos_tab, a->qkv); p.o = const_cast<void*>(static_cast<const void*>(a->o)); p.lse = const_cast<float*>(a->lse);
    if (ROT) p.sin_tab = cos_or_stub(a->sin_tab, a->qkv);
    p.B = a->B; p.N = a->N; p.E = a->E; p.heads = a->heads;
    p.nkeep = nkeep;
    LNX_CHECK(!(nkeep && a->drop_mask), "%s: nkeep (compact rows) and the attention-probability mask (laid out by full rows) do not go together", who);
    p.qtiles = cdiv(a->N, BT);
    if (a->drop_mask) {
        p.amask = a->drop_mask; p.a_inv_keep = a->drop_inv_keep; p.Np = p.qtiles * BT;
    }
    family = attn_family(a->dtype, a->N, hd, a->drop_mask != nullptr);
    g_last_attn.store(family, std::memory_order_relaxed);
    return 0;
}

}

extern "C" int lnx_rope_cos_table(const float* freqs, int heads, int H, int W, float* cos_out, float* dsin_out, void* stream) {
    return rope_table_hd(freqs, heads, 64, H, W, cos_out, dsin_out, (hipStream_t)stream, "lnx_rope_cos_table");
}

extern "C" int lnx_rope_cos_table_hd(const float* freqs, int heads, int head_dim, int H, int W, float* cos_out, float* dsin_out, void* stream) {
    return rope_table_hd(freqs, heads, head_dim, H, W, cos_out, dsin_out, (hipStream_t)stream, "lnx_rope_cos_table_hd");
}

extern "C" int lnx_rope_cossin_table_hd(const float* freqs, int heads, int head_dim, int H, int W, float* cos_out, float* sin_out, float* dsin_out, void* stream) {
    return rope_table_hd(freqs, heads, head_dim, H, W, cos_out, dsin_out, (hipStream_t)stream, "lnx_rope_cossin_table_hd", sin_out);
}

extern "C" int lnx_rope_cos_tables(const lnx_rope_table* t, int n, void* stream) {
    LNX_CHECK(t && n > 0, "lnx_rope_cos_tables: bad arguments");
    for (int i = 0; i < n; ++i) LNX_CHECK(t[i].freqs && t[i].cos_out && t[i].heads > 0 && t[i].H > 0 && t[i].W > 0, "lnx_rope_cos_tables: bad table");
    for (int i = 0; i < n; ++i)
        LNX_CHECK(t[i].head_dim == 0 || hd_ok(t[i].head_dim), "lnx_rope_cos_tables: head_dim %d is not supported (32, 64 or 128)", t[i].head_dim);
    for (int i = 0; i < n; ++i) {
        LNX_CHECK(t[i].rope_mode == LNX_ROPE_COS || t[i].rope_mode == LNX_ROPE_ROTATE, "lnx_rope_cos_tables: bad rope_mode %d", t[i].rope_mode);
        LNX_CHECK(t[i].rope_mode != LNX_ROPE_ROTATE || t[i].sin_out, "lnx_rope_cos_tables: a LNX_ROPE_ROTATE table needs sin_out");
    }
    for (const int hd : {64, 32, 128}) {
        std::vector<lnx_rope_table> g;
        for (int i = 0; i < n; ++i)
            if ((t[i].head_dim ? t[i].head_dim : 64) == hd) g.push_back(t[i]);
        const int ng = (int)g.size();
        for (int i0 = 0; i0 < ng; i0 += LNX_ROPE_TABLES_MAX) {
// ... 76 lines not shown
            g_freq_stream = st;
        } else {
            with_hd(hd, [&](auto hdc) {
                hipLaunchKernelGGL(rope_freqs_reduce_kernel<decltype(hdc)::value>, dim3(a->heads), dim3(1024), 0, st, p.fpart, a->B, a->heads, per_bh, a->dfreqs, nkeep);
            });
        }
    }
    LNX_LAUNCH_CHECK();
    return 0;
}

extern "C" int lnx_attn_fwd_compact(const lnx_attn_args* a, const int* nkeep, void* stream) {
    LNX_CHECK(a && a->qkv && a->o, "lnx_attn_fwd: null operand");
    LNX_CHECK(a->rope_mode == LNX_ROPE_COS || a->rope_mode == LNX_ROPE_ROTATE, "lnx_attn_fwd: bad rope_mode %d", a->rope_mode);
    return a->rope_mode == LNX_ROPE_ROTATE ? attn_fwd_launch<true>(a, nkeep, stream) : attn_fwd_launch<false>(a, nkeep, stream);
}
extern "C" int lnx_attn_fwd(const lnx_attn_args* a, void* stream) { return lnx_attn_fwd_compact(a, nullptr, stream); }

extern "C" int lnx_attn_bwd_compact(const lnx_attn_bwd_args* a, const int* nkeep, int64_t freq_ws_floats, void* stream) {
    LNX_CHECK(a && a->qkv && a->o && a->lse && a->d_o && a->dqkv && a->delta, "lnx_attn_bwd: null operand");
    LNX_CHECK(a->rope_mode == LNX_ROPE_COS || a->rope_mode == LNX_ROPE_ROTATE, "lnx_attn_bwd: bad rope_mode %d", a->rope_mode);
    return a->rope_mode == LNX_ROPE_ROTATE ? attn_bwd_launch<true>(a, nkeep, freq_ws_floats, stream) : attn_bwd_launch<false>(a, nkeep, freq_ws_floats, stream);
}
extern "C" int lnx_attn_bwd_sized(const lnx_attn_bwd_args* a, int64_t freq_ws_floats, void* stream) { return lnx_attn_bwd_compact(a, nullptr, freq_ws_floats, stream); }

extern "C" int lnx_attn_bwd(const lnx_attn_bwd_args* a, void* stream) { return lnx_attn_bwd_sized(a, 0, stream); }

extern "C" int lnx_attn_dispatch(int dtype, int N, int head_dim, int has_drop_mask) {
    const int hd = head_dim ? head_dim : 64;
    if ((dtype != LNX_F32 && dtype != LNX_BF16) || N <= 0 || !hd_ok(hd)) return -1;
    return attn_family(dtype, N, hd, has_drop_mask != 0);
}

extern "C" int lnx_last_attn_kernel(void) { return g_last_attn.load(std::memory_order_relaxed); }

extern "C" int lnx_last_attn_bwd_launches(void) { return g_last_bwd_launches.load(std::memory_order_relaxed); }

extern "C" int lnx_attn_bwd_flush(void* stream) { return freq_flush((hipStream_t)stream); }

extern "C" int lnx_attn_bwd_discard(void) {
    const int n = g_freq_n;
    g_freq_n = 0;
    return n;
}
```

### linnaeus_amd/csrc/elementwise.hip

```cpp
#include "common.hpp"
#include "../../include/lnx.h"

namespace {

inline int ew_grid(int64_t work_items, int per_block) {
    int64_t g = (work_items + per_block - 1) / per_block;
    if (g > 4096) g = 4096;
    if (g < 1) g = 1;
    return (int)g;
}

template <typename T>
__global__ __launch_bounds__(256) void im2col_stem_kernel(const float* __restrict__ x, T* __restrict__ out, int B, int Cin, int H, int W, int ldp) {
    const int Ho = H >> 2, Wo = W >> 2;
    const int units_per_row = ldp >> 2;
    const int64_t total = (int64_t)B * Ho * Wo * units_per_row;
    for (int64_t i = (int64_t)blockIdx.x * blockDim.x + threadIdx.x; i < total; i += (int64_t)gridDim.x * blockDim.x) {
        const int u = (int)(i % units_per_row);
        const int64_t row = i / units_per_row;
        const int wo = (int)(row % Wo);
        const int64_t t = row / Wo;
        const int ho = (int)(t % Ho);
        const int b = (int)(t / Ho);
        float4 v = make_float4(0.f, 0.f, 0.f, 0.f);
// ... 135 lines not shown
            const T* zp = z + (int64_t)m * C + 4 * tc;
            const float z0 = to_f(zp[0]), z1 = to_f(zp[1]), z2 = to_f(zp[2]), z3 = to_f(zp[3]);
            T* o = dz + (int64_t)m * C + 4 * tc;
            o[0] = from_f<T>(s * gm.x * gv.x);
            o[1] = from_f<T>(s * gm.y * gv.y);
            o[2] = from_f<T>(s * gm.z * gv.z);
            o[3] = from_f<T>(s * gm.w * gv.w);
            acc.x += s * gv.x * z0;
            acc.y += s * gv.y * z1;
            acc.z += s * gv.z * z2;
            acc.w += s * gv.w * z3;
        }
        *reinterpret_cast<float4*>(red + tr * C + 4 * tc) = acc;
    }
    __syncthreads();
    for (int c = threadIdx.x; c < C; c += 256) {
        float t = 0.f;
        for (int r = 0; r < rows_pb; ++r) t += red[r * C + c];
        if (part) part[(int64_t)blockIdx.x * C + c] = t;
        else atomicAdd(dgamma + c, t);
    }
}

__global__ __launch_bounds__(256) void fill_rows_kernel(const float* __restrict__ vec, float* __restrict__ out, int64_t ldout, RowMap map, int M, int C) {
    const int c4n = C >> 2;
    const int64_t total = (int64_t)M * c4n;
    for (int64_t i = (int64_t)blockIdx.x * blockDim.x + threadIdx.x; i < total; i += (int64_t)gridDim.x * blockDim.x) {
        const int m = (int)(i / c4n);
        const int c = (int)(i % c4n) * 4;
        *reinterpret_cast<float4*>(out + map_row(map, m) * ldout + c) = *reinterpret_cast<const float4*>(vec + c);
    }
}

__global__ __launch_bounds__(256) void colsum_rows_kernel(const float* __restrict__ in, int64_t ldin, RowMap map, float* __restrict__ out, int M, int C,
                                                          int rows_per_block) {
    const int m0 = blockIdx.x * rows_per_block;
    const int m1 = min(M, m0 + rows_per_block);
    for (int c = threadIdx.x; c < C; c += 256) {
        float t = 0.f;
        for (int m = m0; m < m1; ++m) t += in[map_row(map, m) * ldin + c];
        atomicAdd(out + c, t);
    }
}

__global__ __launch_bounds__(256) void agg2_fwd_kernel(const float* __restrict__ a, const float* __restrict__ b, const float* __restrict__ w2,
                                                       const float* __restrict__ bias1, float* __restrict__ out, int64_t total) {
    const float w0 = w2[0], w1 = w2[1], bb = bias1[0];
    for (int64_t i = (int64_t)blockIdx.x * blockDim.x + threadIdx.x; i < total; i += (int64_t)gridDim.x * blockDim.x) out[i] = w0 * a[i] + w1 * b[i] + bb;
}

__global__ __launch_bounds__(256) void agg2_bwd_kernel(const float* __restrict__ dout, const float* __restrict__ a, const float* __restrict__ b,
                                                       const float* __restrict__ w2, float* __restrict__ da, float* __restrict__ db_, float* __restrict__ dw2,
                                                       float* __restrict__ dbias1, int64_t total) {
    __shared__ float red[3][4];
    const float w0 = w2[0], w1 = w2[1];
    float s0 = 0.f, s1 = 0.f, s2 = 0.f;
    for (int64_t i = (int64_t)blockIdx.x * blockDim.x + threadIdx.x; i < total; i += (int64_t)gridDim.x * blockDim.x) {
        const float d = dout[i];
        da[i] = w0 * d;
        db_[i] = w1 * d;
        s0 += d * a[i];
        s1 += d * b[i];
        s2 += d;
    }
    s0 = wave_sum(s0);
    s1 = wave_sum(s1);
// ... 329 lines not shown
    LNX_CHECK(M > 0 && C > 0 && C % 4 == 0 && C <= 1024, "lnx_layerscale_bwd: bad shape M=%d C=%d (C is a multiple of 4, at most 1024)", M, C);
    const int c4n = C / 4;
    const int rows_pb = 256 / c4n;
    const int grid = layerscale_bwd_grid(M, C);
    const size_t lds = (size_t)rows_pb * C * sizeof(float);
    hipStream_t st = (hipStream_t)stream;
    const int rps = rows_per_sample > 0 ? rows_per_sample : 1;
    float* part = nullptr;
    if (deterministic()) {
        LNX_CHECK(ws != nullptr && ws_floats >= (int64_t)grid * C,
                  "lnx_layerscale_bwd: deterministic mode needs lnx_layerscale_bwd_ws with ws of lnx_layerscale_bwd_ws_floats(M=%d, C=%d) = %lld floats (got %lld): "
                  "without it dgamma is summed by float atomics", M, C, (long long)grid * C, (long long)(ws ? ws_floats : 0));
        part = ws;
    }
    DISPATCH_T(dtype, hipLaunchKernelGGL((layerscale_bwd_kernel<T>), dim3(grid), dim3(256), lds, st, g, (const T*)z, gamma, rowscale, rps, (T*)dz, dgamma, part, M, C));
    if (part) launch_fold(part, grid, C, C, dgamma, st);
    LNX_LAUNCH_CHECK();
    return 0;
}

extern "C" int lnx_layerscale_bwd(const float* g, const void* z, int dtype, const float* gamma, const float* rowscale, int rows_per_sample, void* dz,
                                  float* dgamma, int M, int C, void* stream) {
    return lnx_layerscale_bwd_ws(g, z, dtype, gamma, rowscale, rows_per_sample, dz, dgamma, M, C, nullptr, 0, stream);
}

extern "C" int lnx_fill_rows(const float* vec, float* out, int64_t ldout, lnx_rowmap map, int M, int C, void* stream) {
    LNX_CHECK(vec && out && M > 0 && C % 4 == 0, "lnx_fill_rows: bad arguments");
    hipLaunchKernelGGL(fill_rows_kernel, dim3(ew_grid((int64_t)M * (C / 4), 256)), dim3(256), 0, (hipStream_t)stream, vec, out, ldout,
                       RowMap{map.group, map.pad, map.off}, M, C);
    LNX_LAUNCH_CHECK();
    return 0;
}

extern "C" int lnx_colsum_rows(const float* in, int64_t ldin, lnx_rowmap map, float* out, int M, int C, void* stream) {
    LNX_CHECK(in && out && M > 0 && C > 0, "lnx_colsum_rows: bad arguments");
    const int rpb = deterministic() ? M : 32;
    hipLaunchKernelGGL(colsum_rows_kernel, dim3(cdiv(M, rpb)), dim3(256), 0, (hipStream_t)stream, in, ldin, RowMap{map.group, map.pad, map.off}, out, M, C, rpb);
    LNX_LAUNCH_CHECK();
    return 0;
}

extern "C" int lnx_agg2_fwd(const float* a, const float* b, const float* w2, const float* bias1, float* out, int M, int C, void* stream) {
    LNX_CHECK(a && b && w2 && bias1 && out, "lnx_agg2_fwd: null operand");
    const int64_t total = (int64_t)M * C;
    hipLaunchKernelGGL(agg2_fwd_kernel, dim3(ew_grid(total, 256)), dim3(256), 0, (hipStream_t)stream, a, b, w2, bias1, out, total);
    LNX_LAUNCH_CHECK();
    return 0;
}

extern "C" int lnx_agg2_bwd(const float* dout, const float* a, const float* b, const float* w2, float* da, float* db_, float* dw2, float* dbias1, int M,
                            int C, void* stream) {
    LNX_CHECK(dout && a && b && w2 && da && db_ && dw2 && dbias1, "lnx_agg2_bwd: null operand");
    const int64_t total = (int64_t)M * C;
    int grid = ew_grid(total, 1024);
    if (grid > 256) grid = 256;
    if (deterministic()) grid = 1;
    hipLaunchKernelGGL(agg2_bwd_kernel, dim3(grid), dim3(256), 0, (hipStream_t)stream, dout, a, b, w2, da, db_, dw2, dbias1, total);
    LNX_LAUNCH_CHECK();
    return 0;
}

extern "C" int lnx_pack_meta(const float* meta, int width, int off, int dim, void* out, int dtype, int B, void* stream) {
    LNX_CHECK(meta && out && dim > 0 && dim <= 16 && off >= 0 && off + dim <= width, "lnx_pack_meta: bad arguments width=%d off=%d dim=%d", width, off, dim);
    hipStream_t st = (hipStream_t)stream;
    DISPATCH_T(dtype, hipLaunchKernelGGL((pack_meta_kernel<T>), dim3(cdiv(B * 16, 256)), dim3(256), 0, st, meta, width, off, dim, (T*)out, B));
    LNX_LAUNCH_CHECK();
// ... 18 lines not shown
```

### linnaeus_amd/csrc/plan.cpp

```cpp
#include <hip/hip_runtime.h>
#include <stdlib.h>
#include <string.h>

#include <mutex>
#include <atomic>
#include <string>
#include <vector>

#include "../../include/lnx.h"

void lnx_set_error(const char* fmt, ...);

#define RUN(expr)                  \
    do {                           \
        const int rc_ = (expr);    \
        if (rc_ != 0) return rc_;  \
    } while (0)
#define FAIL(...)                   \
    do {                            \
        lnx_set_error(__VA_ARGS__); \
        return 1;                   \
    } while (0)
#define HIPRUN(expr)                                                         \
    do {                                                                     \
// ... 123 lines not shown
    float inv_keep = 1.0f;
    int64_t dmask_bytes = 0;
    const unsigned char* amask = nullptr;
    float a_inv_keep = 1.0f;
    int64_t amask_bytes = 0;
    hipStream_t side = nullptr;
    hipEvent_t ev_fork = nullptr, ev_meta = nullptr, ev_bfork[2] = {nullptr, nullptr}, ev_bjoin[2] = {nullptr, nullptr};
    hipStream_t wgs = nullptr;
    bool wgs_on = true;
    bool meta_forked[2] = {false, false};
    int meta_mode = 1;
    bool meta_chain = true;
    bool chain_ok[2] = {false, false};
    bool dy8_ready = false;
    hipEvent_t ev_wf[4] = {nullptr, nullptr, nullptr, nullptr}, ev_wj[4] = {nullptr, nullptr, nullptr, nullptr};
    bool profile = false;
    bool profile_spans = false;
    struct Span { hipEvent_t e0, e1; int cls; double work, bytes; };
    std::vector<Span> spans;
    std::vector<hipEvent_t> ev_pool;
    size_t ev_used = 0;

    template <typename U> U* at(int64_t off) const { return reinterpret_cast<U*>(ws + off); }
    const float* drop_ptr(int call) const {
        if (last_drop == nullptr || call < 0 || !mask_host[call]) return nullptr;
        return last_drop + (int64_t)call * c.batch;
    }
    int* droplists = nullptr;
    bool compact_now = false;
    bool compact_conv_now = false;
    bool last_cls_now = false;
    bool trunk_valid = false;
    bool last_cls(int s, int i) const { return last_cls_now && s == 1 && i + 1 == (int)rope[1].size(); }
    const int* drop_list(int call) const {
        if (!compact_now || droplists == nullptr || drop_ptr(call) == nullptr) return nullptr;
        return droplists + (int64_t)call * LNX_DROP_LIST_INTS(c.batch);
    }
};

static std::atomic<int> g_drop_compact{-1};
static std::atomic<long long> g_compact_branches{0};
extern "C" int lnx_set_drop_compact(int on) {
    const int was = g_drop_compact.exchange(on < 0 ? -1 : (on ? 1 : 0));
    return was;
}
extern "C" int64_t lnx_drop_compact_branches(void) { return (int64_t)g_compact_branches.load(std::memory_order_relaxed); }
static std::atomic<long long> g_compact_conv_blocks{0};
extern "C" int64_t lnx_drop_compact_conv_blocks(void) { return (int64_t)g_compact_conv_blocks.load(std::memory_order_relaxed); }
static std::atomic<int> g_last_cls{-1};
static std::atomic<long long> g_last_cls_blocks{0};
extern "C" int lnx_set_last_cls(int on) { return g_last_cls.exchange(on < 0 ? -1 : (on ? 1 : 0)); }
extern "C" int64_t lnx_last_cls_blocks(void) { return (int64_t)g_last_cls_blocks.load(std::memory_order_relaxed); }

namespace {

bool env_set(const char* name) { return getenv(name) != nullptr; }
bool env_off(const char* name) {
    const char* e = getenv(name);
    return e != nullptr && atoi(e) == 0;
}

OpW make_w(lnx_plan* p, int param, int N, int K, bool want_t, int mode = LNX_PREP_CAST, int P = 0, bool f32 = false) {
    OpW w;
    w.param = param;
    w.N = N;
    w.K = K;
    w.f32 = f32 || p->esz == 4;
    const int epv = w.f32 ? 4 : 8;
    w.ld = (int)align_up(K, epv);
    if (K < 16) w.ld = 16;
    w.ld_t = want_t ? (int)align_up(N, epv) : 0;
    w.mode = mode;
    w.P = P;
    return w;
}

void build_params(lnx_plan* p) {
    const lnx_mformer_cfg& c = p->c;
    const int* D = c.dims;
    const int B = c.batch;
    char b[128];
    auto add = [&](const std::string& name, int64_t numel, int seg) {
        p->names.push_back(name);
        p->numel.push_back(numel);
        p->seg.push_back((signed char)seg);
// ... 1137 lines not shown
}

double rope_block_flops(int B, int N, int C, int hid) {
    const double M = (double)B * N;
    return 2.0 * M * C * (3.0 * C + C + 2.0 * hid) + 4.0 * B * (double)N * N * C;
}

Compact compact_of(const lnx_plan* p, int call, int M, int C, int N) {
    Compact cl;
    const int* list = p->drop_list(call);
    if (list == nullptr || fp8_rows(p, M, C) || p->dmask || p->amask) return cl;
    cl.nkeep = list; cl.m_dev = list + 1; cl.perm = list + 2; cl.inv = list + 2 + p->c.batch; cl.rps = N;
    return cl;
}

int rope_block_fwd(const Ctx& c, int s, int i, float* xout) {
    lnx_plan* p = c.p;
    RopeBlk& k = p->rope[s][i];
    const int B = p->c.batch, C = p->c.dims[2 + s], heads = p->c.rope_heads[s], hid = p->c.mlp_hidden[s];
    const int N = p->Ntok[s], M = B * N, E = p->E;
    const float* xin = c.at<float>(k.xin);
    const bool lc = p->last_cls(s, i);
    const Compact ca = compact_of(p, p->drop_attn[s][i], M, C, N), cm = lc ? Compact() : compact_of(p, p->drop_mlp[s][i], M, C, N);
    g_compact_branches.fetch_add((ca ? 1 : 0) + (cm ? 1 : 0), std::memory_order_relaxed);
    p->resident[2 + s] = i;
    Timed span(c, 8, rope_block_flops(B, N, C, hid));
    const bool f8 = fp8_rows(p, M, C);
    void* a8 = f8 ? c.at<void>(p->o_a8) : nullptr;
    void* a8s = f8 ? c.at<void>(p->o_a8s) : nullptr;
    RUN(ln_fwd(c, M, C, 1e-5f, xin, LNX_F32, C, IDM, k.n1w, k.n1b, c.at<void>(k.n1), c.dt, C, IDM, nullptr, 0, c.at<float>(k.mean1), c.at<float>(k.rstd1), a8, a8s, ca));
    lnx_gemm_args g = gemm_base(c, M, 3 * C, C, c.at<void>(k.n1), C, c.wptr(k.qkv), k.qkv.ld, c.at<void>(k.qkvbuf), 3 * C, false);
    g.bias = p->P[k.qkvb]; g.m_dev = ca.m_dev;
    RUN(linear_fwd(c, g, k.qkv, p->o_a8, p->o_a8s));
    lnx_attn_args a;
    memset(&a, 0, sizeof a);
    a.dtype = c.dt; a.B = B; a.N = N; a.E = E; a.heads = heads; a.head_dim = C / heads;
    a.qkv = c.at<void>(k.qkvbuf); a.cos_tab = c.at<float>(k.cos); a.o = c.at<void>(k.o); a.lse = c.at<float>(k.lse);
    if (p->c.rope_mode == LNX_ROPE_ROTATE) {
        a.rope_mode = LNX_ROPE_ROTATE; a.sin_tab = c.at<float>(k.dsin);
    }
    if (p->amask) {
        a.drop_mask = p->amask + k.dm_attn; a.drop_inv_keep = p->a_inv_keep;
    }
    {
        Timed t(c, 2, 4.0 * B * (double)N * N * C);
        RUN(lnx_attn_fwd_compact(&a, ca.nkeep, c.st));
    }
    if (lc) {
        const int64_t ldt = (int64_t)N * C;
        const lnx_rowmap clsrow = {1, N - 1, 0};
        g_last_cls_blocks.fetch_add(1, std::memory_order_relaxed);
        g = gemm_base(c, B, C, C, c.at<void>(k.o), ldt, c.wptr(k.proj), k.proj.ld, c.at<float>(k.xmid), ldt, true);
        g.bias = p->P[k.projb]; g.rowscale = p->drop_ptr(p->drop_attn[s][i]); g.rows_per_sample = 1; g.res = xin; g.ldres = ldt;
        g.m_dev = ca.nkeep; g.perm = ca.perm;
        RUN(gemm_nt_t(c, &g));
        if (ca) RUN(lnx_copy_dropped_rows(xin, c.at<float>(k.xmid), ldt, ca.perm, ca.nkeep, B, 1, C, c.st));
        RUN(ln_fwd(c, B, C, 1e-5f, c.at<float>(k.xmid), LNX_F32, C, clsrow, k.n2w, k.n2b, c.at<void>(k.n2), c.dt, C, IDM, nullptr, 0, c.at<float>(k.mean2), c.at<float>(k.rstd2)));
        g = gemm_base(c, B, hid, C, c.at<void>(k.n2), C, c.wptr(k.fc1), k.fc1.ld, c.at<void>(k.act), hid, false);
        g.bias = p->P[k.fc1b]; g.act = LNX_ACT_GELU_D; g.c2 = c.at<void>(k.hpre); g.ldc2 = hid;
        if (p->c.inference) {
            g.act = LNX_ACT_GELU; g.c2 = nullptr; g.ldc2 = 0;
        }
        RUN(gemm_nt_t(c, &g));
        g = gemm_base(c, B, C, hid, c.at<void>(k.act), hid, c.wptr(k.fc2), k.fc2.ld, xout, ldt, true);
        g.bias = p->P[k.fc2b]; g.rowscale = p->drop_ptr(p->drop_mlp[s][i]); g.rows_per_sample = 1; g.res = c.at<float>(k.xmid); g.ldres = ldt;
        RUN(gemm_nt_t(c, &g));
        return 0;
    }
// ... 38 lines not shown
int plan_forward(lnx_plan* p, const float* x, const float* meta, const float* drop_scales, const unsigned char* drop_mask, float* feats, float* logits,
                 void* stream) {
    if (!p || !p->bound) FAIL("lnx_plan_forward: plan is not bound");
    if (!x) FAIL("lnx_plan_forward: null input");
    const lnx_mformer_cfg& cf = p->c;
    if (cf.n_meta > 0 && !meta) FAIL("lnx_plan_forward: metadata components are configured but meta is NULL");
    if (cf.n_tasks > 0 && !logits) FAIL("lnx_plan_forward: logits buffer is NULL");
    Ctx c{p, stream, cf.dtype};
    const int B = cf.batch;
    const int* D = cf.dims;
    p->last_drop = drop_scales;
    p->mask_host.assign(p->n_drop, 0);
    if (drop_scales && drop_mask)
        for (int i = 0; i < p->n_drop; ++i) p->mask_host[i] = drop_mask[i];
    p->last_meta = meta;

    RUN(lnx_prep_weights(c.at<lnx_prep_desc>(p->o_descs), (int)p->n_descs_t, (int)p->prep_blocks, cf.dtype, stream));
    if (p->n_descs_f > 0)
        RUN(lnx_prep_weights(c.at<lnx_prep_desc>(p->o_descs) + p->n_descs_t, (int)p->n_descs_f, (int)p->prep_blocks_f, LNX_F32, stream));
    if (cf.fp8)
        for (int s = 0; s < 2; ++s)
            for (auto& k : p->rope[s]) {
                for (const OpW* w : {&k.qkv, &k.fc1, &k.fc2})
                    RUN(lnx_quantize_mxfp8(p->P[w->param], LNX_F32, w->K, w->N, w->K, c.at<void>(w->off8), w->K, c.at<void>(w->off8s), stream));
                for (const OpW* w : {&k.proj, &k.fc1, &k.fc2})
                    if (w->off8ts)
                        RUN(lnx_quantize_mxfp8(c.wtptr(*w), LNX_BF16, w->ld_t, w->K, w->N, c.at<void>(w->off8t), w->N, c.at<void>(w->off8ts), stream));
            }

    {
        const int sw = g_last_cls.load(std::memory_order_relaxed);
        const bool on = sw < 0 ? !env_off("LNX_LAST_CLS") : sw != 0;
        p->last_cls_now = on && cf.rope_depths[1] > 0 && cf.fp8 == 0 && !p->dmask && !p->amask;
    }
    p->compact_now = false;
    p->compact_conv_now = false;
    {
        const int sw = g_drop_compact.load(std::memory_order_relaxed);
        const bool on = sw < 0 ? !env_off("LNX_DROP_COMPACT") : sw != 0;
        if (on && !cf.inference && p->n_drop > 0 && drop_scales && !p->dmask && !p->amask) {
            std::vector<unsigned char> want(p->n_drop, 0);
            std::vector<int> rps(p->n_drop, 1);
            bool any = false, any_conv = false;
            if (!env_off("LNX_DROP_COMPACT_CONV"))
                for (int s = 0; s < 2; ++s)
                    for (size_t i = 0; i < p->conv[s].size(); ++i) {
                        const int call = p->drop_conv[s][i];
                        if (p->mask_host[call] && p->conv[s][i].fused && p->conv[s][i].fused_ln) {
                            want[call] = 1;
                            rps[call] = p->H[s] * p->W[s];
                            any = any_conv = true;
                        }
                    }
            for (int s = 0; s < 2; ++s)
                for (size_t i = 0; i < p->rope[s].size(); ++i)
                    for (const int call : {p->drop_attn[s][i], p->drop_mlp[s][i]})
                        if (p->mask_host[call] && !fp8_rows(p, B * p->Ntok[s], D[2 + s]) && !(p->last_cls((int)s, (int)i) && call == p->drop_mlp[s][i])) {
                            want[call] = 1;
                            rps[call] = p->Ntok[s];
                            any = true;
                        }
            if (any) {
                if (p->droplists == nullptr) HIPRUN(hipMalloc((void**)&p->droplists, (size_t)p->n_drop * LNX_DROP_LIST_INTS(B) * sizeof(int)));
                RUN(lnx_drop_partition(drop_scales, p->n_drop, B, want.data(), rps.data(), p->droplists, stream));
                p->compact_now = true;
                p->compact_conv_now = any_conv;
// ... 210 lines not shown
    if (!have_dy) {
        if (cm) RUN(lnx_scale_cast_compact(g, C, p->drop_ptr(p->drop_mlp[s][i]), N, cm.perm, cm.m_dev, sC, c.dt, C, M, C, c.st));
        else RUN(lnx_scale_cast(g, C, tm, p->drop_ptr(p->drop_mlp[s][i]), rps, sC, c.dt, C, Mb, C, c.st));
    }
    if (p->dmask) RUN(lnx_dropout_mul(sC, c.dt, p->dmask + k.dm_fc2, p->inv_keep, M, C, c.st));
    RUN(wfork(0));
    RUN(wgrad(cw, Mb, C, hid, sC, C, c.at<void>(k.act), hid, k.fc2.param, k.fc2b, hid, 0, 0, cm.m_dev));
    RUN(wdone(0));
    lnx_gemm_args a = gemm_base(c, Mb, hid, C, sC, C, c.wtptr(k.fc2), k.fc2.ld_t, sA, hid, false);
    a.m_dev = cm.m_dev;
    a.act = fp8_rows(p, M, C) ? LNX_ACT_GELU_BWD : LNX_ACT_MUL_AUX; a.aux = c.at<void>(k.hpre); a.ldaux = hid;
    const bool qpass = env_set("LNX_FP8_DGRAD_QPASS");
    const bool mx_dgrad = c.dt == LNX_BF16 && fp8_rows(p, M, C) && k.fc2.off8ts != 0 && k.proj.off8ts != 0 && !p->dmask && C % 128 == 0 && !qpass;
    RUN(linear_dgrad(c, a, k.fc2, !(have_dy && p->dy8_ready), p->o_a8, p->o_a8s, p->o_h8, p->o_h8s));
    p->dy8_ready = false;
    if (p->dmask) RUN(lnx_dropout_mul(sA, c.dt, p->dmask + k.dm_hid, p->inv_keep, M, hid, c.st));
    RUN(wfork(1));
    RUN(wgrad(cw, Mb, hid, C, sA, hid, c.at<void>(k.n2), C, k.fc1.param, k.fc1b, C, 0, 1, cm.m_dev));
    RUN(wdone(1));
    a = gemm_base(c, Mb, C, hid, sA, hid, c.wtptr(k.fc1), k.fc1.ld_t, sD, C, false);
    a.m_dev = cm.m_dev;
    RUN(linear_dgrad(c, a, k.fc1, false, p->o_h8, p->o_h8s));
    RUN(wjoin(0));
    Dx2 d2;
    d2.p = sC; d2.rowscale = p->drop_ptr(p->drop_attn[s][i]); d2.rps = rps; d2.inv = ca.inv; d2.nkeep = ca.nkeep;
    if (mx_dgrad) {
        d2.p8 = c.at<void>(p->o_a8); d2.p8s = c.at<void>(p->o_a8s);
    }
    RUN(ln_bwd(c, Mb, C, sD, c.dt, C, IDM, c.at<float>(k.xmid), LNX_F32, ldo, IDM, k.n2w, k.n2b, c.at<float>(k.mean2), c.at<float>(k.rstd2), g, g, LNX_F32, ldo, false, d2, cm));
    if (p->dmask) RUN(lnx_dropout_mul(sC, c.dt, p->dmask + k.dm_proj, p->inv_keep, M, C, c.st));
    RUN(wfork(2));
    RUN(wgrad(cw, Mb, C, C, sC, C, c.at<void>(k.o), ldo, k.proj.param, k.projb, C, 0, 2, pj_mdev));
    RUN(wdone(2));
    if (lc) HIPRUN(hipMemsetAsync(sD, 0, (size_t)M * C * p->esz, (hipStream_t)c.st));
    a = gemm_base(c, Mb, C, C, sC, C, c.wtptr(k.proj), k.proj.ld_t, sD, ldo, false);
    a.m_dev = pj_mdev;
    RUN(linear_dgrad(c, a, k.proj, !mx_dgrad, p->o_a8, p->o_a8s));
    RUN(wjoin(1));
    lnx_attn_bwd_args ab;
    memset(&ab, 0, sizeof ab);
    ab.dtype = c.dt; ab.B = B; ab.N = N; ab.E = E; ab.heads = heads; ab.head_dim = C / heads;
    ab.qkv = c.at<void>(k.qkvbuf); ab.cos_tab = c.at<float>(k.cos); ab.o = c.at<void>(k.o); ab.lse = c.at<float>(k.lse);
    ab.d_o = sD; ab.dqkv = sA; ab.freq_ws = c.at<float>(p->o_gcos); ab.delta = c.at<float>(p->o_delta);
    if (p->freq_defer && E < N) {
        if (p->freq_pending == FREQ_DEFER_SLOTS) {
            RUN(lnx_attn_bwd_flush(c.st));
            p->freq_pending = 0;
        }
        ab.freq_ws = c.at<float>(p->o_gcos) + (int64_t)p->freq_pending * p->gcos_floats;
        ab.defer_freqs = 1;
        ++p->freq_pending;
    }
    ab.dsin_tab = c.at<float>(k.dsin); ab.dfreqs = p->G[k.freqs];
    if (p->c.rope_mode == LNX_ROPE_ROTATE) {
        ab.rope_mode = LNX_ROPE_ROTATE; ab.sin_tab = c.at<float>(k.dsin); ab.dsin_tab = nullptr; ab.grid_w = p->W[2 + s];
    }
    if (p->amask) {
        ab.drop_mask = p->amask + k.dm_attn; ab.drop_inv_keep = p->a_inv_keep;
    }
    {
        Timed t(c, 3, 14.0 * B * (double)N * N * C);
        RUN(lnx_attn_bwd_compact(&ab, ca.nkeep, p->gcos_floats, c.st));
    }
    RUN(wfork(3));
    RUN(wgrad(cw, M, 3 * C, C, sA, 3 * C, c.at<void>(k.n1), C, k.qkv.param, k.qkvb, C, 0, 3, ca.m_dev));
    RUN(lnx_gemm_tn_flush(cw.st));
    RUN(wdone(3));
    RUN(wjoin(2));
    void* dn1 = (ca || cprev) ? sD : sC;
    a = gemm_base(c, M, C, 3 * C, sA, 3 * C, c.wtptr(k.qkv), k.qkv.ld_t, dn1, C, false);
    a.m_dev = ca.m_dev;
    RUN(gemm_nt_t(c, &a));
    Dx2 d1;
    if (prev_runs) {
// ... 488 lines not shown
```

### linnaeus_amd/model.py

```python
from __future__ import annotations

import ctypes as C
import math
import os
from collections import OrderedDict
from typing import Any, Dict, List, Optional, Sequence

import torch
import torch.nn as nn

from . import _lib as L
from .heads import configure_classification_heads
from .registry import register_model

_DTYPES = {"bf16": L.BF16, "bfloat16": L.BF16, "fp32": L.F32, "float32": L.F32}


class _Cfg(C.Structure):
    _fields_ = [
        ("dtype", C.c_int), ("batch", C.c_int), ("img_h", C.c_int), ("img_w", C.c_int), ("in_chans", C.c_int),
        ("dims", C.c_int * 4), ("conv_depths", C.c_int * 2), ("rope_depths", C.c_int * 2), ("rope_heads", C.c_int * 2),
        ("mlp_hidden", C.c_int * 2), ("n_meta", C.c_int), ("meta_dims", C.c_int * 8), ("only_last_cls", C.c_int),
        ("n_tasks", C.c_int), ("task_classes", C.c_int * 16), ("inference", C.c_int), ("recompute", C.c_int), ("fp8", C.c_int),
        ("rope_mode", C.c_int),
# ... 265 lines not shown
            "supports_module_prefix": True,
            "strict": False,
        }

    def set_compute_dtype(self, name: str) -> None:
        name = name.lower()
        self._fp8 = name in ("fp8", "mxfp8")
        self._dtype_code = L.BF16 if self._fp8 else _DTYPES[name]
        self.release_plans()

    def set_deterministic(self, on: bool) -> None:
        L.set_deterministic(bool(on))
        self.release_plans()

    @staticmethod
    def set_drop_compact(on: Optional[bool]) -> int:
        return int(L.lib().lnx_set_drop_compact(-1 if on is None else int(bool(on))))

    @staticmethod
    def drop_compact_branches() -> int:
        return int(L.lib().lnx_drop_compact_branches())

    @staticmethod
    def drop_compact_conv_blocks() -> int:
        return int(L.lib().lnx_drop_compact_conv_blocks())

    @staticmethod
    def set_last_cls(on: Optional[bool]) -> int:
        return int(L.lib().lnx_set_last_cls(-1 if on is None else int(bool(on))))

    @staticmethod
    def last_cls_blocks() -> int:
        return int(L.lib().lnx_last_cls_blocks())

    def set_wgrad_stream(self, on: bool) -> None:
        self._wgrad_stream = bool(on)
        for st in self._plans.values():
            if st.get("handle") is not None and L.lib().lnx_plan_set_wgrad_stream(st["handle"], int(self._wgrad_stream)) < 0:
                L.check(1, "lnx_plan_set_wgrad_stream")

    def set_meta_stream(self, mode: int) -> None:
        if mode not in (0, 1, 2):
            raise ValueError(f"meta stream mode {mode!r}: 0 (launch stream), 1 (side stream) or 2 (weight-gradient stream)")
        self._meta_stream = int(mode)
        for st in self._plans.values():
            if st.get("handle") is not None and L.lib().lnx_plan_set_meta_stream(st["handle"], self._meta_stream) < 0:
                L.check(1, "lnx_plan_set_meta_stream")

    def _destroy_plan(self, st) -> None:
        if st.get("destroyed"):
            return
        st["destroyed"] = True
        try:
            L.lib().lnx_plan_destroy(st["handle"])
        finally:
            st["handle"] = None
            st["ws"] = None
            st["dl_buf"] = st["dl_views"] = None
            st["dropout_masks"] = st["attn_dropout_masks"] = None
            st["saved_inputs"] = None

    def release_plans(self) -> None:
        if torch.cuda.is_available() and self._plans:
            torch.cuda.synchronize()
        for st in list(self._plans.values()):
            self._destroy_plan(st)
# ... 579 lines not shown
```

### linnaeus_amd/ops.py

```python
from __future__ import annotations

import ctypes as C
from typing import Optional, Tuple

import torch

from . import _lib as L
from ._lib import F32, BF16

_TORCH_DT = {F32: torch.float32, BF16: torch.bfloat16}


def code_of(t: torch.Tensor) -> int:
    if t.dtype == torch.float32:
        return F32
    if t.dtype == torch.bfloat16:
        return BF16
    raise L.LnxError(f"unsupported tensor dtype {t.dtype}")


def torch_dtype(code: int) -> torch.dtype:
    return _TORCH_DT[code]


# ... 283 lines not shown
    return out


def rope_cossin_table(freqs, H, W):
    heads, half = freqs.shape[1], freqs.shape[2]
    cos = torch.empty(H * W, heads, half, device=freqs.device, dtype=torch.float32)
    sin = torch.empty_like(cos)
    L.check(L.lib().lnx_rope_cossin_table_hd(_p(freqs), heads, 2 * half, H, W, _p(cos), _p(sin), None, _stream()), "lnx_rope_cossin_table_hd")
    return cos, sin


def rope_cos_tables(entries):
    arr = (L.RopeTable * len(entries))()
    for t, (freqs, H, W, out, dsin, *rest) in zip(arr, entries):
        t.freqs, t.cos_out, t.dsin_out = _p(freqs), _p(out), _p(dsin) if dsin is not None else None
        t.heads, t.H, t.W, t.head_dim = freqs.shape[1], H, W, 2 * freqs.shape[2]
        if rest and rest[0] is not None:
            t.rope_mode, t.sin_out = L.ROPE_ROTATE, _p(rest[0])
    L.check(L.lib().lnx_rope_cos_tables(arr, len(entries), _stream()), "lnx_rope_cos_tables")


def attn_bwd_ws_floats(B, N, heads, head_dim=64):
    fn = L.lib().lnx_attn_bwd_ws_floats_hd
    fn.restype = C.c_int64
    return int(fn(B, N, heads, head_dim))


def _head_dim(qkv, heads, head_dim):
    if head_dim is not None:
        return int(head_dim)
    return qkv.shape[-1] // (3 * heads) if qkv.dim() >= 2 and qkv.shape[-1] % (3 * heads) == 0 else 64


def attn_fwd(qkv, cos_tab, o, lse, B, N, E, heads, *, drop_mask=None, drop_rate=0.0, head_dim=None, sin_tab=None, nkeep=None):
    a = L.AttnArgs()
    if sin_tab is not None:
        a.rope_mode, a.sin_tab = L.ROPE_ROTATE, _p(sin_tab)
    a.dtype, a.B, a.N, a.E, a.heads = code_of(qkv), B, N, E, heads
    a.head_dim = _head_dim(qkv, heads, head_dim)
    a.qkv, a.cos_tab, a.o, a.lse = _p(qkv), _p(cos_tab), _p(o), _p(lse)
    if drop_mask is not None:
        a.drop_mask, a.drop_inv_keep = _p(drop_mask), 1.0 / (1.0 - drop_rate)
    if nkeep is not None:
        L.check(L.lib().lnx_attn_fwd_compact(C.byref(a), _p(nkeep), _stream()), "lnx_attn_fwd_compact")
        return
    L.check(L.lib().lnx_attn_fwd(C.byref(a), _stream()), "lnx_attn_fwd")


def attn_bwd(qkv, cos_tab, o, lse, d_o, dqkv, delta, B, N, E, heads, *, dsin=None, dfreqs=None, drop_mask=None, drop_rate=0.0, defer_freqs=False,
             head_dim=None, sin_tab=None, grid_w=0, nkeep=None):
    a = L.AttnBwdArgs()
    if sin_tab is not None:
        a.rope_mode, a.sin_tab, a.grid_w, a.dfreqs = L.ROPE_ROTATE, _p(sin_tab), int(grid_w), _p(dfreqs) if dfreqs is not None else None
    a.dtype, a.B, a.N, a.E, a.heads = code_of(qkv), B, N, E, heads
    a.head_dim = _head_dim(qkv, heads, head_dim)
    a.qkv, a.cos_tab, a.o, a.lse = _p(qkv), _p(cos_tab), _p(o), _p(lse)
    ws = torch.empty(max(attn_bwd_ws_floats(B, N, heads, a.head_dim), 1), device=qkv.device, dtype=torch.float32)
    a.d_o, a.dqkv, a.freq_ws, a.delta = _p(d_o), _p(dqkv), _p(ws), _p(delta)
    if dsin is not None:
        a.dsin_tab, a.dfreqs = _p(dsin), _p(dfreqs)
    if drop_mask is not None:
        a.drop_mask, a.drop_inv_keep = _p(drop_mask), 1.0 / (1.0 - drop_rate)
    a.defer_freqs = int(bool(defer_freqs))
    if nkeep is not None:
        L.check(L.lib().lnx_attn_bwd_compact(C.byref(a), _p(nkeep), C.c_int64(ws.numel()), _stream()), "lnx_attn_bwd_compact")
        return ws
    L.check(L.lib().lnx_attn_bwd_sized(C.byref(a), C.c_int64(ws.numel()), _stream()), "lnx_attn_bwd")
    return ws


def attn_bwd_flush():
    L.check(L.lib().lnx_attn_bwd_flush(_stream()), "lnx_attn_bwd_flush")


def im2col_stem(x, patches):
    B, Cin, H, W = x.shape
    L.check(L.lib().lnx_im2col_stem(_p(x), B, Cin, H, W, _p(patches), code_of(patches), patches.stride(0), _stream()), "lnx_im2col_stem")


def stem_fwd(x, w, bias, ln_w, ln_b, y, *, patches=None, pre=None, mean=None, rstd=None, eps=1e-6):
    a = L.StemArgs()
    a.x, a.w, a.bias, a.ln_w, a.ln_b = _p(x), _p(w), _p(bias), _p(ln_w), _p(ln_b)
    a.patches, a.pre, a.y, a.mean, a.rstd = _p(patches), _p(pre), _p(y), _p(mean), _p(rstd)
    a.B, a.Cin, a.H, a.W = x.shape
# ... 21 lines not shown
    def __init__(self, lists: torch.Tensor, B: int):
        self.lists, self.B = lists, B

    def nkeep(self, c):
        return self.lists[c, 0:1]

    def m_dev(self, c):
        return self.lists[c, 1:2]

    def perm(self, c):
        return self.lists[c, 2:2 + self.B]

    def inv(self, c):
        return self.lists[c, 2 + self.B:2 + 2 * self.B]


def drop_partition(scales: torch.Tensor, rows_per_sample=None, call_mask=None) -> DropLists:
    n, B = scales.shape
    lists = torch.zeros((n, L.drop_list_ints(B)), device=scales.device, dtype=torch.int32)
    rps = (C.c_int * n)(*[int(r) for r in rows_per_sample]) if rows_per_sample is not None else None
    mask = bytes(bytearray(int(bool(m)) for m in call_mask)) if call_mask is not None else None
    L.check(L.lib().lnx_drop_partition(_p(scales.contiguous()), n, B, mask, rps, _p(lists), _stream()), "lnx_drop_partition")
    return DropLists(lists, B)


def layerscale_bwd(g, z, gamma, rowscale, rows_per_sample, dz, dgamma, M, Cc):
    if L.is_deterministic():
        ws = torch.empty(max(int(L.lib().lnx_layerscale_bwd_ws_floats(M, Cc)), 1), device=g.device, dtype=torch.float32)
        L.check(L.lib().lnx_layerscale_bwd_ws(_p(g), _p(z), code_of(z), _p(gamma), _p(rowscale), rows_per_sample, _p(dz), _p(dgamma), M, Cc, _p(ws),
                                              C.c_int64(ws.numel()), _stream()), "lnx_layerscale_bwd_ws")
        return
    L.check(L.lib().lnx_layerscale_bwd(_p(g), _p(z), code_of(z), _p(gamma), _p(rowscale), rows_per_sample, _p(dz), _p(dgamma), M, Cc, _stream()),
            "lnx_layerscale_bwd")


def fill_rows(vec, out, ldout, row_map, M, Cc):
    L.check(L.lib().lnx_fill_rows(_p(vec), _p(out), C.c_int64(ldout), _map(row_map), M, Cc, _stream()), "lnx_fill_rows")


def colsum_rows(inp, ldin, row_map, out, M, Cc):
    L.check(L.lib().lnx_colsum_rows(_p(inp), C.c_int64(ldin), _map(row_map), _p(out), M, Cc, _stream()), "lnx_colsum_rows")


def agg2_fwd(a, b, w2, bias1, out, M, Cc):
    L.check(L.lib().lnx_agg2_fwd(_p(a), _p(b), _p(w2), _p(bias1), _p(out), M, Cc, _stream()), "lnx_agg2_fwd")


def agg2_bwd(dout, a, b, w2, da, db, dw2, dbias1, M, Cc):
    L.check(L.lib().lnx_agg2_bwd(_p(dout), _p(a), _p(b), _p(w2), _p(da), _p(db), _p(dw2), _p(dbias1), M, Cc, _stream()), "lnx_agg2_bwd")


def pack_meta(meta, off, dim, out):
    L.check(L.lib().lnx_pack_meta(_p(meta), meta.shape[1], off, dim, _p(out), code_of(out), meta.shape[0], _stream()), "lnx_pack_meta")


def convmlp_fwd(ln, w1, b1, w2, b2, gamma, x, out, *, rowscale=None, rows_per_sample=0, z=None, y=None, ln_w=None, ln_b=None, ln_eps=1e-6,
                ln_out=None, mean=None, rstd=None, perm=None, m_dev=None):
    a = L.ConvMlpArgs()
    src = ln if y is None else y
    a.dtype, a.M, a.C = code_of(src), src.shape[0], src.shape[1]
    a.ln, a.w1, a.b1, a.w2, a.b2, a.gamma = _p(ln), _p(w1), _p(b1), _p(w2), _p(b2), _p(gamma)
    a.rowscale, a.rows_per_sample, a.x, a.out, a.z = _p(rowscale), rows_per_sample, _p(x), _p(out), _p(z)
    a.y, a.ln_w, a.ln_b, a.ln_eps, a.ln_out, a.mean, a.rstd = _p(y), _p(ln_w), _p(ln_b), ln_eps, _p(ln_out), _p(mean), _p(rstd)
    a.perm, a.m_dev = _p(perm), _p(m_dev)
    L.check(L.lib().lnx_convmlp_fwd(C.byref(a), _stream()), "lnx_convmlp_fwd")
    return out
# ... 244 lines not shown
```

Measured before the change: 14280 images/sec.

## Restrict last-block attention to the CLS query row in forward and backward

Adds a q_rows parameter to the attention forward and backward kernels so that the final transformer block, whose output only feeds the classification token, computes attention for the CLS query row alone. The backward pass skips query tiles past q_rows and iterates only over the live query rows when accumulating dK/dV. The full memset of the d_o buffer is dropped and only the dQ columns are zeroed. This removes query-side work in the last block, but it depends on correctly zeroing the unused gradient rows and on the kernel family supporting q_rows.

```diff
diff --git a/include/lnx.h b/include/lnx.h
--- a/include/lnx.h
+++ b/include/lnx.h
@@ -257,6 +257,7 @@
     const unsigned char* drop_mask;
     float drop_inv_keep;
     int head_dim;
+    int q_rows;
     int rope_mode;
     const float* sin_tab;
 } lnx_attn_args;
@@ -279,6 +280,7 @@
     float* dfreqs;
     int defer_freqs;
     int head_dim;
+    int q_rows;
     int rope_mode;
     const float* sin_tab;
     int grid_w;
@@ -294,6 +296,7 @@
 enum { LNX_ATTN_KERNEL_NONE = 0, LNX_ATTN_KERNEL_RES4 = 1 , LNX_ATTN_KERNEL_RES8 = 2 ,
        LNX_ATTN_KERNEL_TILED4 = 3 , LNX_ATTN_KERNEL_TILED8 = 4  };
 int lnx_attn_dispatch(int dtype, int N, int head_dim, int has_drop_mask);
+int lnx_attn_q_rows_ok(int dtype, int N, int head_dim, int has_drop_mask);
 int lnx_last_attn_kernel(void);
 int lnx_last_attn_bwd_launches(void);
 
@@ -332,6 +335,8 @@
 int64_t lnx_drop_compact_conv_blocks(void);
 int lnx_set_last_cls(int on);
 int64_t lnx_last_cls_blocks(void);
+int lnx_set_last_cls_q(int on);
+int64_t lnx_last_cls_q_blocks(void);
 
 int lnx_layerscale_bwd(const float* g, const void* z, int dtype, const float* gamma, const float* rowscale,
                        int rows_per_sample, void* dz, float* dgamma, int M, int C, void* stream);
@@ -342,6 +347,8 @@
 int lnx_dropout_mul(void* x, int dtype, const unsigned char* mask, float inv_keep, int M, int C, void* stream);
 int lnx_dropout_residual(const void* z, int z_dtype, const unsigned char* mask, float inv_keep, const float* rowscale, int rows_per_sample,
                          const float* res, float* out, int M, int C, void* stream);
+
+int lnx_zero_cols(void* x, int64_t ld_bytes, int64_t width_bytes, int M, void* stream);
 
 int lnx_fill_rows(const float* vec, float* out, int64_t ldout, lnx_rowmap map, int M, int C, void* stream);
 int lnx_layerscale_bwd_ws(const float* g, const void* z, int dtype, const float* gamma, const float* rowscale, int rows_per_sample, void* dz,
diff --git a/linnaeus_amd/_lib.py b/linnaeus_amd/_lib.py
--- a/linnaeus_amd/_lib.py
+++ b/linnaeus_amd/_lib.py
@@ -376,6 +376,11 @@
         if hasattr(_lib, "lnx_last_cls_blocks"):
             _lib.lnx_set_last_cls.argtypes = [C.c_int]
             _lib.lnx_last_cls_blocks.restype = C.c_int64
+        if hasattr(_lib, "lnx_last_cls_q_blocks"):
+            _lib.lnx_zero_cols.argtypes = [C.c_void_p, C.c_int64, C.c_int64, C.c_int, C.c_void_p]
+            _lib.lnx_set_last_cls_q.argtypes = [C.c_int]
+            _lib.lnx_last_cls_q_blocks.restype = C.c_int64
+            _lib.lnx_attn_q_rows_ok.argtypes = [C.c_int, C.c_int, C.c_int, C.c_int]
         if hasattr(_lib, "lnx_plan_forward_tail"):
             _lib.lnx_plan_forward_tail.argtypes = [C.c_void_p, C.c_void_p, C.c_void_p, C.c_void_p, C.c_void_p]
             _lib.lnx_plan_trunk_valid.argtypes = [C.c_void_p]
@@ -421,8 +426,8 @@
     "lnx_gemm_nt", "lnx_last_nt_kernel", "lnx_nt_kernel_launches", "lnx_nt_dispatch", "lnx_gemm_tn", "lnx_gemm_tn_query", "lnx_gemm_tn_flush", "lnx_gemm_tn_discard", "lnx_amax", "lnx_quantize_fp8", "lnx_gemm_nt_fp8", "lnx_quantize_mxfp8", "lnx_gemm_nt_mxfp8", "lnx_dropout_mul", "lnx_dropout_residual", "lnx_plan_dropout_bytes", "lnx_plan_set_dropout", "lnx_plan_attn_dropout_bytes", "lnx_plan_set_attn_dropout",
     "lnx_layernorm_fwd", "lnx_layernorm_bwd", "lnx_layernorm_bwd_flush", "lnx_layernorm_bwd_discard", "lnx_layernorm_fwd_query", "lnx_layernorm_bwd_query",
     "lnx_dwconv7_fwd", "lnx_dwconv7_fwd_kept", "lnx_dwconv7_wgrad", "lnx_dwconv7_wgrad_kept", "lnx_dwconv7_wgrad_ws_floats",
-    "lnx_gemm_nt_group_ok", "lnx_gemm_nt_group", "lnx_rope_cos_table", "lnx_rope_cos_table_hd", "lnx_rope_cossin_table_hd", "lnx_rope_cos_tables", "lnx_attn_bwd_ws_floats", "lnx_attn_bwd_ws_floats_hd", "lnx_attn_fwd", "lnx_attn_bwd", "lnx_attn_bwd_sized", "lnx_attn_fwd_compact", "lnx_attn_bwd_compact", "lnx_attn_bwd_flush", "lnx_attn_bwd_discard", "lnx_attn_dispatch", "lnx_last_attn_kernel", "lnx_last_attn_bwd_launches",
-    "lnx_im2col_stem", "lnx_scale_cast", "lnx_scale_cast_compact", "lnx_drop_partition", "lnx_copy_dropped_rows", "lnx_set_drop_compact", "lnx_drop_compact_branches", "lnx_drop_compact_conv_blocks", "lnx_set_last_cls", "lnx_last_cls_blocks", "lnx_layerscale_bwd", "lnx_layerscale_bwd_ws", "lnx_layerscale_bwd_ws_floats", "lnx_layerscale_apply_wgrad", "lnx_fill_rows", "lnx_colsum_rows",
+    "lnx_gemm_nt_group_ok", "lnx_gemm_nt_group", "lnx_rope_cos_table", "lnx_rope_cos_table_hd", "lnx_rope_cossin_table_hd", "lnx_rope_cos_tables", "lnx_attn_bwd_ws_floats", "lnx_attn_bwd_ws_floats_hd", "lnx_attn_fwd", "lnx_attn_bwd", "lnx_attn_bwd_sized", "lnx_attn_fwd_compact", "lnx_attn_bwd_compact", "lnx_attn_bwd_flush", "lnx_attn_bwd_discard", "lnx_attn_dispatch", "lnx_attn_q_rows_ok", "lnx_last_attn_kernel", "lnx_last_attn_bwd_launches",
+    "lnx_im2col_stem", "lnx_scale_cast", "lnx_scale_cast_compact", "lnx_drop_partition", "lnx_copy_dropped_rows", "lnx_set_drop_compact", "lnx_drop_compact_branches", "lnx_drop_compact_conv_blocks", "lnx_set_last_cls", "lnx_last_cls_blocks", "lnx_set_last_cls_q", "lnx_last_cls_q_blocks", "lnx_layerscale_bwd", "lnx_layerscale_bwd_ws", "lnx_layerscale_bwd_ws_floats", "lnx_layerscale_apply_wgrad", "lnx_zero_cols", "lnx_fill_rows", "lnx_colsum_rows",
     "lnx_agg2_fwd", "lnx_agg2_bwd", "lnx_pack_meta", "lnx_meta_heads_supported", "lnx_meta_heads_fwd", "lnx_meta_heads_bwd", "lnx_meta_heads_bwd_part_floats", "lnx_prep_weights", "lnx_prep_blocks", "lnx_softce", "lnx_softce_multi", "lnx_taxonomy_rows", "lnx_stem_fwd", "lnx_stem_fwd_ok", "lnx_adamw_blocks", "lnx_grad_sumsq", "lnx_adamw_step", "lnx_ademamix_step", "lnx_sgd_step", "lnx_optim_launches", "lnx_grad_sumsq_guarded", "lnx_adamw_step_guarded", "lnx_ademamix_step_guarded", "lnx_sgd_step_guarded", "lnx_muon_layout", "lnx_muon_step", "lnx_muon_launches", "lnx_muon_partition", "lnx_muon_orthogonalize", "lnx_muon_apply_packed", "lnx_gradnorm_sumsq", "lnx_gradnorm_update",
     "lnx_metrics_table_sizes", "lnx_metrics_update", "lnx_predict", "lnx_resize_taps", "lnx_resize_coeffs", "lnx_preprocess_scratch_bytes", "lnx_preprocess", "lnx_hier_loss_fwd", "lnx_hier_loss_bwd",
     "lnx_hier_refine_fwd", "lnx_hier_refine_bwd", "lnx_hier_refine_launches",
@@ -531,7 +536,7 @@
     _fields_ = [
         ("dtype", C.c_int), ("B", C.c_int), ("N", C.c_int), ("E", C.c_int), ("heads", C.c_int),
         ("qkv", C.c_void_p), ("cos_tab", C.c_void_p), ("o", C.c_void_p), ("lse", C.c_void_p),
-        ("drop_mask", C.c_void_p), ("drop_inv_keep", C.c_float), ("head_dim", C.c_int),
+        ("drop_mask", C.c_void_p), ("drop_inv_keep", C.c_float), ("head_dim", C.c_int), ("q_rows", C.c_int),
         ("rope_mode", C.c_int), ("sin_tab", C.c_void_p),
     ]
 
@@ -542,7 +547,7 @@
         ("qkv", C.c_void_p), ("cos_tab", C.c_void_p), ("o", C.c_void_p), ("lse", C.c_void_p),
         ("d_o", C.c_void_p), ("dqkv", C.c_void_p), ("freq_ws", C.c_void_p), ("delta", C.c_void_p),
         ("drop_mask", C.c_void_p), ("drop_inv_keep", C.c_float),
-        ("dsin_tab", C.c_void_p), ("dfreqs", C.c_void_p), ("defer_freqs", C.c_int), ("head_dim", C.c_int),
+        ("dsin_tab", C.c_void_p), ("dfreqs", C.c_void_p), ("defer_freqs", C.c_int), ("head_dim", C.c_int), ("q_rows", C.c_int),
         ("rope_mode", C.c_int), ("sin_tab", C.c_void_p), ("grid_w", C.c_int),
     ]
 
diff --git a/linnaeus_amd/csrc/api.cpp b/linnaeus_amd/csrc/api.cpp
--- a/linnaeus_amd/csrc/api.cpp
+++ b/linnaeus_amd/csrc/api.cpp
@@ -19,7 +19,7 @@
 }
 
 extern "C" const char* lnx_last_error(void) { return g_err; }
-extern "C" int lnx_version(void) { return 120; }
+extern "C" int lnx_version(void) { return 121; }
 extern "C" int lnx_device_cus(void) {
     int dev = 0;
     if (hipGetDevice(&dev) != hipSuccess) return -1;
diff --git a/linnaeus_amd/csrc/attention.hip b/linnaeus_amd/csrc/attention.hip
--- a/linnaeus_amd/csrc/attention.hip
+++ b/linnaeus_amd/csrc/attention.hip
@@ -361,6 +361,7 @@
     int W = 1;
     float* fwave = nullptr;
     const int* nkeep = nullptr;
+    int qrows = 0;
 };
 
 template <int HD = 64> __device__ __forceinline__ float* freq_wave_slot(const AttnP& p) {
@@ -461,7 +462,7 @@
 template <typename T, int HD = 64, bool ROT = false>
 __device__ __forceinline__ void dq_epilogue(const AttnP& p, const f32x4_t (&dq)[HD / 16], const T* __restrict__ qb, int64_t ld, int b, int head, int q, int s, int g,
                                             float scale, float* fl, float* fw) {
-    const int qc = min(q, p.N - 1);
+    const int qc = min(q, p.qrows - 1);
     const T* qraw = qb + (int64_t)qc * ld;
     const float* cpr = p.cos_tab + ((int64_t)max(qc - p.E, 0) * p.heads + head) * (HD / 2);
     const float* sxp = p.dsin + ((int64_t)max(qc - p.E, 0) * p.heads + head) * (HD / 2);
@@ -503,7 +504,7 @@
             dy[dt][0] = b2.x; dy[dt][1] = b2.y;
         }
     }
-    const bool row = q < p.N, img = row && q >= p.E;
+    const bool row = q < p.qrows, img = row && q >= p.E;
     T* dqp = reinterpret_cast<T*>(p.dqkv) + ((int64_t)b * p.N + qc) * ld + head * HD;
     float oq[ND][4];
 #pragma unroll
@@ -547,7 +548,7 @@
 
     const int q = qt * (16 * NW) + wave * 16 + s;
     uint4 qf[(AT<T, HD>::NKK)];
-    load_row_frag<T, true, HD, ROT>(qf, qb, ld, q, p.N, p.E, g, p.cos_tab, p.heads, head, scale, p.sin_tab);
+    load_row_frag<T, true, HD, ROT>(qf, qb, ld, q, p.qrows, p.E, g, p.cos_tab, p.heads, head, scale, p.sin_tab);
 
     f32x4_t oacc[HD / 16];
 #pragma unroll
@@ -626,8 +627,8 @@
         for (int dt = 0; dt < HD / 16; ++dt)
 #pragma unroll
             for (int r = 0; r < 4; ++r) ov[dt][r] = oacc[dt][r] * inv;
-        store_row<T, HD>(reinterpret_cast<T*>(p.o) + ((int64_t)b * p.N + min(q, p.N - 1)) * C + head * HD, ov, g, q < p.N);
-        if (q < p.N && g == 0 && p.lse) p.lse[((int64_t)b * p.heads + head) * p.N + q] = m_run + logf(l_tot);
+        store_row<T, HD>(reinterpret_cast<T*>(p.o) + ((int64_t)b * p.N + min(q, p.qrows - 1)) * C + head * HD, ov, g, q < p.qrows);
+        if (q < p.qrows && g == 0 && p.lse) p.lse[((int64_t)b * p.heads + head) * p.N + q] = m_run + logf(l_tot);
     }
 }
 
@@ -652,17 +653,21 @@
     const T* ob = reinterpret_cast<const T*>(p.o) + (int64_t)b * p.N * C + head * HD;
     const float scale = attn_scale<HD>();
 
+    if (qt * (16 * NW) >= p.qrows) {
+        if (p.E < p.N && threadIdx.x < HD) p.fpart[(int64_t)blockIdx.x * HD + threadIdx.x] = 0.f;
+        return;
+    }
     __shared__ float fl[HD];
     float* fw = freq_wave_slot<HD>(p);
     if (threadIdx.x < HD) fl[threadIdx.x] = 0.f;
     const int q = qt * (16 * NW) + wave * 16 + s;
     uint4 qf[(AT<T, HD>::NKK)], dof[(AT<T, HD>::NKK)];
-    load_row_frag<T, true, HD, ROT>(qf, qb, ld, q, p.N, p.E, g, p.cos_tab, p.heads, head, scale, p.sin_tab);
-    load_row_frag<T, false, HD>(dof, dob, C, q, p.N, p.E, g, nullptr, p.heads, head, 1.0f);
+    load_row_frag<T, true, HD, ROT>(qf, qb, ld, q, p.qrows, p.E, g, p.cos_tab, p.heads, head, scale, p.sin_tab);
+    load_row_frag<T, false, HD>(dof, dob, C, q, p.qrows, p.E, g, nullptr, p.heads, head, 1.0f);
     float dl = 0.f;
     {
         uint4 of[(AT<T, HD>::NKK)];
-        load_row_frag<T, false, HD>(of, ob, C, q, p.N, p.E, g, nullptr, p.heads, head, 1.0f);
+        load_row_frag<T, false, HD>(of, ob, C, q, p.qrows, p.E, g, nullptr, p.heads, head, 1.0f);
 #pragma unroll
         for (int kk = 0; kk < AT<T, HD>::NKK; ++kk) {
             Vec16<T> a, bb;
@@ -673,9 +678,9 @@
         }
     }
     const float delta = group_sum(dl);
-    const float lse_raw = p.lse[((int64_t)b * p.heads + head) * p.N + min(q, p.N - 1)];
-    const float lse = RowExp<T>::prep(q < p.N ? lse_raw : 0.f);
-    if (q < p.N && g == 0) p.delta[((int64_t)b * p.heads + head) * p.N + q] = delta;
+    const float lse_raw = p.lse[((int64_t)b * p.heads + head) * p.N + min(q, p.qrows - 1)];
+    const float lse = RowExp<T>::prep(q < p.qrows ? lse_raw : 0.f);
+    if (q < p.qrows && g == 0) p.delta[((int64_t)b * p.heads + head) * p.N + q] = delta;
 
     f32x4_t dq[HD / 16];
 #pragma unroll
@@ -768,29 +773,30 @@
         dk[i] = f32x4_t{0.f, 0.f, 0.f, 0.f};
         dv[i] = f32x4_t{0.f, 0.f, 0.f, 0.f};
     }
-    const int nqt = (p.N + BT - 1) / BT;
+    const int NQ = p.qrows;
+    const int nqt = (NQ + BT - 1) / BT;
     TileFetch<T, true, 64 * NW, HD, ROT> fq;
     TileFetch<T, false, 64 * NW, HD> fdo;
     const int stl = threadIdx.x & (BT - 1);
     float l_n, d_n;
-    fq.fetch(qb, ld, 0, p.N, p.E, p.cos_tab, p.heads, head, p.sin_tab);
-    fdo.fetch(dob, C, 0, p.N, p.E, nullptr, p.heads, head);
-    l_n = p.lse[statbase + min(stl, p.N - 1)];
-    d_n = p.delta[statbase + min(stl, p.N - 1)];
+    fq.fetch(qb, ld, 0, NQ, p.E, p.cos_tab, p.heads, head, p.sin_tab);
+    fdo.fetch(dob, C, 0, NQ, p.E, nullptr, p.heads, head);
+    l_n = p.lse[statbase + min(stl, NQ - 1)];
+    d_n = p.delta[statbase + min(stl, NQ - 1)];
     for (int qt = 0; qt < nqt; ++qt) {
         __syncthreads();
-        fq.template commit<true, true>(qimg, qtr, qt * BT, p.N, p.E, scale);
-        fdo.template commit<true, true>(doimg, dotr, qt * BT, p.N, p.E, 1.0f);
+        fq.template commit<true, true>(qimg, qtr, qt * BT, NQ, p.E, scale);
+        fdo.template commit<true, true>(doimg, dotr, qt * BT, NQ, p.E, 1.0f);
         if (threadIdx.x < BT) {
             const int qq = qt * BT + threadIdx.x;
-            lse_s[threadIdx.x] = RowExp<T>::prep(qq < p.N ? l_n : 0.f);
-            del_s[threadIdx.x] = qq < p.N ? d_n : 0.f;
+            lse_s[threadIdx.x] = RowExp<T>::prep(qq < NQ ? l_n : 0.f);
+            del_s[threadIdx.x] = qq < NQ ? d_n : 0.f;
         }
         const int nxt = min(qt + 1, nqt - 1) * BT;
-        fq.fetch(qb, ld, nxt, p.N, p.E, p.cos_tab, p.heads, head, p.sin_tab);
-        fdo.fetch(dob, C, nxt, p.N, p.E, nullptr, p.heads, head);
-        l_n = p.lse[statbase + min(nxt + stl, p.N - 1)];
-        d_n = p.delta[statbase + min(nxt + stl, p.N - 1)];
+        fq.fetch(qb, ld, nxt, NQ, p.E, p.cos_tab, p.heads, head, p.sin_tab);
+        fdo.fetch(dob, C, nxt, NQ, p.E, nullptr, p.heads, head);
+        l_n = p.lse[statbase + min(nxt + stl, NQ - 1)];
+        d_n = p.delta[statbase + min(nxt + stl, NQ - 1)];
         __syncthreads();
 #pragma unroll
         for (int h = 0; h < 2; ++h) {
@@ -892,11 +898,11 @@
     stage_all<T, true, true, false, ROT>(kimg, nullptr, kb, ld, npad, p.N, p.E, p.cos_tab, p.heads, head, 1.0f, p.sin_tab);
     stage_all<T, false, false, true>(nullptr, vimg, vb, ld, npad, p.N, p.E, nullptr, p.heads, head, 1.0f);
     __syncthreads();
-    const int nq16 = (p.N + 15) / 16;
+    const int nq16 = (p.qrows + 15) / 16;
     for (int qt = wave; qt < nq16; qt += NW) {
         const int q = qt * 16 + s;
         uint4 qf[AT<T>::NKK];
-        load_row_frag<T, true, 64, ROT>(qf, qb, ld, q, p.N, p.E, g, p.cos_tab, p.heads, head, scale, p.sin_tab);
+        load_row_frag<T, true, 64, ROT>(qf, qb, ld, q, p.qrows, p.E, g, p.cos_tab, p.heads, head, scale, p.sin_tab);
         f32x4_t oacc[4];
 #pragma unroll
         for (int i = 0; i < 4; ++i) oacc[i] = f32x4_t{0.f, 0.f, 0.f, 0.f};
@@ -952,8 +958,8 @@
             for (int dt = 0; dt < 4; ++dt)
 #pragma unroll
                 for (int r = 0; r < 4; ++r) ov[dt][r] = oacc[dt][r] * inv;
-            store_row<T>(reinterpret_cast<T*>(p.o) + ((int64_t)b * p.N + min(q, p.N - 1)) * C + head * HD, ov, g, q < p.N);
-            if (q < p.N && g == 0 && p.lse) p.lse[((int64_t)b * p.heads + head) * p.N + q] = m_run + logf(l_tot);
+            store_row<T>(reinterpret_cast<T*>(p.o) + ((int64_t)b * p.N + min(q, p.qrows - 1)) * C + head * HD, ov, g, q < p.qrows);
+            if (q < p.qrows && g == 0 && p.lse) p.lse[((int64_t)b * p.heads + head) * p.N + q] = m_run + logf(l_tot);
         }
     }
 }
@@ -1003,7 +1009,7 @@
 __device__ __forceinline__ void dq_res_epilogue(const AttnP& p, const f32x4_t (&dq)[4], const float (&qr)[4][4], float (&cr)[4][2], int64_t ld, int b, int head, int q,
                                                 int s, int g, float scale, float* fl, float* fw) {
     constexpr int HD = 64;
-    const int qc = min(q, p.N - 1);
+    const int qc = min(q, p.qrows - 1);
     const float* cpr = p.cos_tab + ((int64_t)max(qc - p.E, 0) * p.heads + head) * 32;
     const float* sxp = p.dsin + ((int64_t)max(qc - p.E, 0) * p.heads + head) * 32;
     const float* syp = sxp + (int64_t)(p.N - p.E) * p.heads * 32;
@@ -1025,7 +1031,7 @@
         dx[dt][0] = a.x; dx[dt][1] = a.y;
         dy[dt][0] = c.x; dy[dt][1] = c.y;
     }
-    const bool row = q < p.N, img = row && q >= p.E;
+    const bool row = q < p.qrows, img = row && q >= p.E;
     T* dqp = reinterpret_cast<T*>(p.dqkv) + ((int64_t)b * p.N + qc) * ld + head * HD;
     float oq[4][4];
 #pragma unroll
@@ -1122,34 +1128,35 @@
     stage_all<T, true, false, true, ROT>(nullptr, kimg, kb, ld, npad, p.N, p.E, p.cos_tab, p.heads, head, 1.0f, p.sin_tab);
     stage_all<T, false, false, true>(nullptr, vimg, vb, ld, npad, p.N, p.E, nullptr, p.heads, head, 1.0f);
     __syncthreads();
-    const int nq16 = (p.N + 15) / 16;
+    const int NQ = p.qrows;
+    const int nq16 = (NQ + 15) / 16;
     for (int qt = wave; qt < nq16; qt += NW) {
         const int q = qt * 16 + s;
-        const int qc = min(q, p.N - 1);
+        const int qc = min(q, NQ - 1);
         uint4 qf[AT<T>::NKK], dof[AT<T>::NKK];
         Chunk<T, true, 64, ROT> cq[AT<T>::NKK];
         Chunk<T, false> cdo[AT<T>::NKK], co[AT<T>::NKK];
 #pragma unroll
         for (int kk = 0; kk < AT<T>::NKK; ++kk) {
             const int d0 = (kk * 4 + g) * AT<T>::EPV;
-            cq[kk].fetch(qb, ld, q, p.N, p.E, d0, p.cos_tab, p.heads, head, p.sin_tab);
-            cdo[kk].fetch(dob, C, q, p.N, p.E, d0, nullptr, p.heads, head);
-            co[kk].fetch(ob, C, q, p.N, p.E, d0, nullptr, p.heads, head);
+            cq[kk].fetch(qb, ld, q, NQ, p.E, d0, p.cos_tab, p.heads, head, p.sin_tab);
+            cdo[kk].fetch(dob, C, q, NQ, p.E, d0, nullptr, p.heads, head);
+            co[kk].fetch(ob, C, q, NQ, p.E, d0, nullptr, p.heads, head);
         }
         const float lse_raw = p.lse[((int64_t)b * p.heads + head) * p.N + qc];
         float qr[4][4], cr[4][2];
         dq_res_prefetch<T, ROT>(qr, cr, p, qb, ld, qc, head, g);
 #pragma unroll
         for (int kk = 0; kk < AT<T>::NKK; ++kk) {
-            qf[kk] = cq[kk].value(q, p.N, p.E, scale);
-            dof[kk] = cdo[kk].value(q, p.N, p.E, 1.0f);
+            qf[kk] = cq[kk].value(q, NQ, p.E, scale);
+            dof[kk] = cdo[kk].value(q, NQ, p.E, 1.0f);
         }
         uint4 of[AT<T>::NKK];
 #pragma unroll
-        for (int kk = 0; kk < AT<T>::NKK; ++kk) of[kk] = co[kk].value(q, p.N, p.E, 1.0f);
+        for (int kk = 0; kk < AT<T>::NKK; ++kk) of[kk] = co[kk].value(q, NQ, p.E, 1.0f);
         const float delta = delta_of_row<T>(dof, of);
-        const float lse = RowExp<T>::prep(q < p.N ? lse_raw : 0.f);
-        if (q < p.N && g == 0) p.delta[((int64_t)b * p.heads + head) * p.N + q] = delta;
+        const float lse = RowExp<T>::prep(q < NQ ? lse_raw : 0.f);
+        if (q < NQ && g == 0) p.delta[((int64_t)b * p.heads + head) * p.N + q] = delta;
         f32x4_t dq[4];
 #pragma unroll
         for (int i = 0; i < 4; ++i) dq[i] = f32x4_t{0.f, 0.f, 0.f, 0.f};
@@ -1196,13 +1203,14 @@
     __shared__ float fl[64];
     float* fw = freq_wave_slot<64>(p);
     if (threadIdx.x < 64) fl[threadIdx.x] = 0.f;
-    stage_all<T, true, false, true, ROT>(nullptr, qimg, qb, ld, npad, p.N, p.E, p.cos_tab, p.heads, head, scale, p.sin_tab);
-    stage_all<T, false, false, true>(nullptr, doimg, dob, C, npad, p.N, p.E, nullptr, p.heads, head, 1.0f);
+    const int NQ = p.qrows, npq = (NQ + 31) & ~31;
+    stage_all<T, true, false, true, ROT>(nullptr, qimg, qb, ld, npq, NQ, p.E, p.cos_tab, p.heads, head, scale, p.sin_tab);
+    stage_all<T, false, false, true>(nullptr, doimg, dob, C, npq, NQ, p.E, nullptr, p.heads, head, 1.0f);
     ATT_T(0);
     for (int i = threadIdx.x; i < nqt * BT; i += blockDim.x) {
-        const float l = p.lse[statbase + min(i, p.N - 1)], d = p.delta[statbase + min(i, p.N - 1)];
-        lse_s[i] = RowExp<T>::prep(i < p.N ? l : 0.f);
-        del_s[i] = i < p.N ? d : 0.f;
+        const float l = p.lse[statbase + min(i, NQ - 1)], d = p.delta[statbase + min(i, NQ - 1)];
+        lse_s[i] = RowExp<T>::prep(i < NQ ? l : 0.f);
+        del_s[i] = i < NQ ? d : 0.f;
     }
     __syncthreads();
     ATT_T(1);
@@ -1231,7 +1239,7 @@
             dv[i] = f32x4_t{0.f, 0.f, 0.f, 0.f};
         }
         ATT_T(2);
-        dkv_res_loop<T>(dk, dv, qimg, doimg, lse_s, del_s, npad, s, g, kf, vf);
+        dkv_res_loop<T>(dk, dv, qimg, doimg, lse_s, del_s, npq, s, g, kf, vf);
         ATT_T(3);
         dkv_epilogue<T, 64, ROT>(p, dk, dv, kb, ld, C, b, head, key, s, g, fl, fw);
         ATT_T(4);
@@ -1283,25 +1291,26 @@
     if (threadIdx.x < 64) fl[threadIdx.x] = 0.f;
     const int row = wave * 16 + s;
     const int ntiles = (p.N + 15) / 16;
-    const bool tile = wave < ntiles;
+    const int NQ = p.qrows, npq = (NQ + 31) & ~31;
+    const bool tile = wave < (NQ + 15) / 16;
     Chunk<T, false> co[AT<T>::NKK];
     {
-        const int total = npad * AT<T>::NCH, i0 = threadIdx.x;
+        const int total = npad * AT<T>::NCH, totq = npq * AT<T>::NCH, i0 = threadIdx.x;
         StageBatch<T, true, ROT, UN> sq, sk;
         StageBatch<T, false, false, UN> sv, sdo;
-        sq.fetch(qb, ld, i0, total, p.N, p.E, p.cos_tab, p.heads, head, p.sin_tab);
+        sq.fetch(qb, ld, i0, totq, NQ, p.E, p.cos_tab, p.heads, head, p.sin_tab);
         sk.fetch(kb, ld, i0, total, p.N, p.E, p.cos_tab, p.heads, head, p.sin_tab);
         sv.fetch(vb, ld, i0, total, p.N, p.E, nullptr, p.heads, head);
-        sdo.fetch(dob, C, i0, total, p.N, p.E, nullptr, p.heads, head);
-        const float l = p.lse[statbase + min(i0, p.N - 1)];
-#pragma unroll
-        for (int kk = 0; kk < AT<T>::NKK; ++kk) co[kk].fetch(ob, C, row, p.N, p.E, (kk * 4 + g) * AT<T>::EPV, nullptr, p.heads, head);
-        sq.template commit<false, true>(nullptr, qimg, i0, total, p.N, p.E, scale);
+        sdo.fetch(dob, C, i0, totq, NQ, p.E, nullptr, p.heads, head);
+        const float l = p.lse[statbase + min(i0, NQ - 1)];
+#pragma unroll
+        for (int kk = 0; kk < AT<T>::NKK; ++kk) co[kk].fetch(ob, C, row, NQ, p.E, (kk * 4 + g) * AT<T>::EPV, nullptr, p.heads, head);
+        sq.template commit<false, true>(nullptr, qimg, i0, totq, NQ, p.E, scale);
         sk.template commit<false, true>(nullptr, kimg, i0, total, p.N, p.E, 1.0f);
         sv.template commit<false, true>(nullptr, vimg, i0, total, p.N, p.E, 1.0f);
-        sdo.template commit<false, true>(nullptr, doimg, i0, total, p.N, p.E, 1.0f);
+        sdo.template commit<false, true>(nullptr, doimg, i0, totq, NQ, p.E, 1.0f);
         if (i0 < nqt * BT) {
-            lse_s[i0] = RowExp<T>::prep(i0 < p.N ? l : 0.f);
+            lse_s[i0] = RowExp<T>::prep(i0 < NQ ? l : 0.f);
             del_s[i0] = 0.f;
         }
     }
@@ -1316,10 +1325,10 @@
         for (int kk = 0; kk < AT<T>::NKK; ++kk) {
             qf[kk] = ld16(qimg + row * AT<T>::TRB + ((kk * 4 + g) << 4));
             dof[kk] = ld16(doimg + row * AT<T>::TRB + ((kk * 4 + g) << 4));
-            of[kk] = co[kk].value(row, p.N, p.E, 1.0f);
+            of[kk] = co[kk].value(row, NQ, p.E, 1.0f);
         }
         delta = delta_of_row<T>(dof, of);
-        if (row < p.N && g == 0) {
+        if (row < NQ && g == 0) {
             p.delta[statbase + row] = delta;
             del_s[row] = delta;
         }
@@ -1328,7 +1337,7 @@
     __syncthreads();
     ATT_T(3);
     if (tile) {
-        const int q = row, qc = min(q, p.N - 1);
+        const int q = row, qc = min(q, NQ - 1);
         float qr[4][4], cr[4][2];
         dq_res_prefetch<T, ROT>(qr, cr, p, qb, ld, qc, head, g);
         const float lse = lse_s[q];
@@ -1355,7 +1364,7 @@
             dk[i] = f32x4_t{0.f, 0.f, 0.f, 0.f};
             dv[i] = f32x4_t{0.f, 0.f, 0.f, 0.f};
         }
-        dkv_res_loop<T>(dk, dv, qimg, doimg, lse_s, del_s, npad, s, g, kf, vf);
+        dkv_res_loop<T>(dk, dv, qimg, doimg, lse_s, del_s, npq, s, g, kf, vf);
         ATT_T(6);
         dkv_epilogue<T, 64, ROT>(p, dk, dv, kb, ld, C, b, head, key, s, g, fl, fw);
         ATT_T(7);
@@ -1521,6 +1530,7 @@
     return tiled_nw8(N) ? LNX_ATTN_KERNEL_TILED8 : LNX_ATTN_KERNEL_TILED4;
 }
 bool is_resident(int family) { return family == LNX_ATTN_KERNEL_RES4 || family == LNX_ATTN_KERNEL_RES8; }
+bool q_rows_family_ok(int family, bool drop) { return !drop && family != LNX_ATTN_KERNEL_TILED8; }
 
 std::atomic<int> g_last_attn{LNX_ATTN_KERNEL_NONE};
 
@@ -1542,6 +1552,7 @@
         constexpr int NW = decltype(nwc)::value;
         constexpr bool DROP = decltype(dropc)::value != 0;
         constexpr size_t lds = AT<T, HD>::FWD_LDS;
+        p.qtiles = cdiv(p.qrows, 16 * NW);
         return attn_launch<attn_fwd_kernel<T, NW, DROP, HD, ROT>>(p.B * p.heads * p.qtiles, 64 * NW, lds, lds, st, p);
     });
 }
@@ -1620,6 +1631,10 @@
         p.amask = a->drop_mask; p.a_inv_keep = a->drop_inv_keep; p.Np = p.qtiles * BT;
     }
     family = attn_family(a->dtype, a->N, hd, a->drop_mask != nullptr);
+    LNX_CHECK(a->q_rows >= 0 && a->q_rows <= a->N, "%s: q_rows %d outside 0..N = %d", who, a->q_rows, a->N);
+    LNX_CHECK(a->q_rows == 0 || q_rows_family_ok(family, a->drop_mask != nullptr),
+              "%s: q_rows = %d, but the kernels this call dispatches to do not take a query limit (lnx_attn_q_rows_ok)", who, a->q_rows);
+    p.qrows = a->q_rows ? a->q_rows : a->N;
     g_last_attn.store(family, std::memory_order_relaxed);
     return 0;
 }
@@ -1762,6 +1777,11 @@
     return attn_family(dtype, N, hd, has_drop_mask != 0);
 }
 
+extern "C" int lnx_attn_q_rows_ok(int dtype, int N, int head_dim, int has_drop_mask) {
+    const int family = lnx_attn_dispatch(dtype, N, head_dim, has_drop_mask);
+    return family > 0 && q_rows_family_ok(family, has_drop_mask != 0) ? 1 : 0;
+}
+
 extern "C" int lnx_last_attn_kernel(void) { return g_last_attn.load(std::memory_order_relaxed); }
 
 extern "C" int lnx_last_attn_bwd_launches(void) { return g_last_bwd_launches.load(std::memory_order_relaxed); }
diff --git a/linnaeus_amd/csrc/elementwise.hip b/linnaeus_amd/csrc/elementwise.hip
--- a/linnaeus_amd/csrc/elementwise.hip
+++ b/linnaeus_amd/csrc/elementwise.hip
@@ -191,6 +191,15 @@
     }
 }
 
+__global__ __launch_bounds__(256) void zero_cols_kernel(unsigned char* __restrict__ x, int64_t ld_bytes, int chunks, int M) {
+    const int64_t total = (int64_t)M * chunks;
+    for (int64_t i = (int64_t)blockIdx.x * blockDim.x + threadIdx.x; i < total; i += (int64_t)gridDim.x * blockDim.x) {
+        const int64_t m = i / chunks;
+        const int c = (int)(i - m * chunks);
+        *reinterpret_cast<uint4*>(x + m * ld_bytes + ((int64_t)c << 4)) = make_uint4(0, 0, 0, 0);
+    }
+}
+
 __global__ __launch_bounds__(256) void colsum_rows_kernel(const float* __restrict__ in, int64_t ldin, RowMap map, float* __restrict__ out, int M, int C,
                                                           int rows_per_block) {
     const int m0 = blockIdx.x * rows_per_block;
@@ -586,6 +595,15 @@
     return 0;
 }
 
+extern "C" int lnx_zero_cols(void* x, int64_t ld_bytes, int64_t width_bytes, int M, void* stream) {
+    LNX_CHECK(x && M > 0 && width_bytes > 0 && width_bytes <= ld_bytes && width_bytes % 16 == 0 && ld_bytes % 16 == 0 && (((uintptr_t)x) & 15) == 0,
+              "lnx_zero_cols: M > 0 rows of 16-byte aligned, whole 16-byte chunks, width_bytes <= ld_bytes");
+    const int chunks = (int)(width_bytes >> 4);
+    hipLaunchKernelGGL(zero_cols_kernel, dim3(ew_grid((int64_t)M * chunks, 256)), dim3(256), 0, (hipStream_t)stream, (unsigned char*)x, ld_bytes, chunks, M);
+    LNX_LAUNCH_CHECK();
+    return 0;
+}
+
 extern "C" int lnx_colsum_rows(const float* in, int64_t ldin, lnx_rowmap map, float* out, int M, int C, void* stream) {
     LNX_CHECK(in && out && M > 0 && C > 0, "lnx_colsum_rows: bad arguments");
     const int rpb = deterministic() ? M : 32;
diff --git a/linnaeus_amd/csrc/plan.cpp b/linnaeus_amd/csrc/plan.cpp
--- a/linnaeus_amd/csrc/plan.cpp
+++ b/linnaeus_amd/csrc/plan.cpp
@@ -179,6 +179,8 @@
     bool last_cls_now = false;
     bool trunk_valid = false;
     bool last_cls(int s, int i) const { return last_cls_now && s == 1 && i + 1 == (int)rope[1].size(); }
+    bool last_cls_q_now = false;
+    bool last_cls_q(int s, int i) const { return last_cls_q_now && last_cls(s, i); }
     const int* drop_list(int call) const {
         if (!compact_now || droplists == nullptr || drop_ptr(call) == nullptr) return nullptr;
         return droplists + (int64_t)call * LNX_DROP_LIST_INTS(c.batch);
@@ -198,6 +200,10 @@
 static std::atomic<long long> g_last_cls_blocks{0};
 extern "C" int lnx_set_last_cls(int on) { return g_last_cls.exchange(on < 0 ? -1 : (on ? 1 : 0)); }
 extern "C" int64_t lnx_last_cls_blocks(void) { return (int64_t)g_last_cls_blocks.load(std::memory_order_relaxed); }
+static std::atomic<int> g_last_cls_q{-1};
+static std::atomic<long long> g_last_cls_q_blocks{0};
+extern "C" int lnx_set_last_cls_q(int on) { return g_last_cls_q.exchange(on < 0 ? -1 : (on ? 1 : 0)); }
+extern "C" int64_t lnx_last_cls_q_blocks(void) { return (int64_t)g_last_cls_q_blocks.load(std::memory_order_relaxed); }
 
 namespace {
 
@@ -1401,8 +1407,11 @@
     lnx_gemm_args g = gemm_base(c, M, 3 * C, C, c.at<void>(k.n1), C, c.wptr(k.qkv), k.qkv.ld, c.at<void>(k.qkvbuf), 3 * C, false);
     g.bias = p->P[k.qkvb]; g.m_dev = ca.m_dev;
     RUN(linear_fwd(c, g, k.qkv, p->o_a8, p->o_a8s));
+    const bool lq = p->last_cls_q(s, i);
+    if (lq) g_last_cls_q_blocks.fetch_add(1, std::memory_order_relaxed);
     lnx_attn_args a;
     memset(&a, 0, sizeof a);
+    a.q_rows = lq ? 1 : 0;
     a.dtype = c.dt; a.B = B; a.N = N; a.E = E; a.heads = heads; a.head_dim = C / heads;
     a.qkv = c.at<void>(k.qkvbuf); a.cos_tab = c.at<float>(k.cos); a.o = c.at<void>(k.o); a.lse = c.at<float>(k.lse);
     if (p->c.rope_mode == LNX_ROPE_ROTATE) {
@@ -1507,6 +1516,9 @@
         const int sw = g_last_cls.load(std::memory_order_relaxed);
         const bool on = sw < 0 ? !env_off("LNX_LAST_CLS") : sw != 0;
         p->last_cls_now = on && cf.rope_depths[1] > 0 && cf.fp8 == 0 && !p->dmask && !p->amask;
+        const int swq = g_last_cls_q.load(std::memory_order_relaxed);
+        const bool onq = swq < 0 ? !env_off("LNX_LAST_CLS_Q") : swq != 0;
+        p->last_cls_q_now = p->last_cls_now && onq && lnx_attn_q_rows_ok(cf.dtype, p->Ntok[1], D[3] / cf.rope_heads[1], 0) != 0;
     }
     p->compact_now = false;
     p->compact_conv_now = false;
@@ -1783,7 +1795,8 @@
     RUN(wfork(2));
     RUN(wgrad(cw, Mb, C, C, sC, C, c.at<void>(k.o), ldo, k.proj.param, k.projb, C, 0, 2, pj_mdev));
     RUN(wdone(2));
-    if (lc) HIPRUN(hipMemsetAsync(sD, 0, (size_t)M * C * p->esz, (hipStream_t)c.st));
+    const bool lq = p->last_cls_q(s, i);
+    if (lc && !lq) HIPRUN(hipMemsetAsync(sD, 0, (size_t)M * C * p->esz, (hipStream_t)c.st));
     a = gemm_base(c, Mb, C, C, sC, C, c.wtptr(k.proj), k.proj.ld_t, sD, ldo, false);
     a.m_dev = pj_mdev;
     RUN(linear_dgrad(c, a, k.proj, !mx_dgrad, p->o_a8, p->o_a8s));
@@ -1791,6 +1804,10 @@
     lnx_attn_bwd_args ab;
     memset(&ab, 0, sizeof ab);
     ab.dtype = c.dt; ab.B = B; ab.N = N; ab.E = E; ab.heads = heads; ab.head_dim = C / heads;
+    if (lq) {
+        ab.q_rows = 1;
+        RUN(lnx_zero_cols(sA, (int64_t)3 * C * p->esz, (int64_t)C * p->esz, M, c.st));
+    }
     ab.qkv = c.at<void>(k.qkvbuf); ab.cos_tab = c.at<float>(k.cos); ab.o = c.at<void>(k.o); ab.lse = c.at<float>(k.lse);
     ab.d_o = sD; ab.dqkv = sA; ab.freq_ws = c.at<float>(p->o_gcos); ab.delta = c.at<float>(p->o_delta);
     if (p->freq_defer && E < N) {
diff --git a/linnaeus_amd/model.py b/linnaeus_amd/model.py
--- a/linnaeus_amd/model.py
+++ b/linnaeus_amd/model.py
@@ -321,6 +321,14 @@
     @staticmethod
     def last_cls_blocks() -> int:
         return int(L.lib().lnx_last_cls_blocks())
+
+    @staticmethod
+    def set_last_cls_q(on: Optional[bool]) -> int:
+        return int(L.lib().lnx_set_last_cls_q(-1 if on is None else int(bool(on))))
+
+    @staticmethod
+    def last_cls_q_blocks() -> int:
+        return int(L.lib().lnx_last_cls_q_blocks())
 
     def set_wgrad_stream(self, on: bool) -> None:
         self._wgrad_stream = bool(on)
diff --git a/linnaeus_amd/ops.py b/linnaeus_amd/ops.py
--- a/linnaeus_amd/ops.py
+++ b/linnaeus_amd/ops.py
@@ -339,8 +339,13 @@
     return qkv.shape[-1] // (3 * heads) if qkv.dim() >= 2 and qkv.shape[-1] % (3 * heads) == 0 else 64
 
 
-def attn_fwd(qkv, cos_tab, o, lse, B, N, E, heads, *, drop_mask=None, drop_rate=0.0, head_dim=None, sin_tab=None, nkeep=None):
+def attn_q_rows_ok(dtype_code, N, head_dim=64, has_drop_mask=False):
+    return bool(L.lib().lnx_attn_q_rows_ok(int(dtype_code), int(N), int(head_dim), int(bool(has_drop_mask))))
+
+
+def attn_fwd(qkv, cos_tab, o, lse, B, N, E, heads, *, drop_mask=None, drop_rate=0.0, head_dim=None, sin_tab=None, nkeep=None, q_rows=0):
     a = L.AttnArgs()
+    a.q_rows = int(q_rows)
     if sin_tab is not None:
         a.rope_mode, a.sin_tab = L.ROPE_ROTATE, _p(sin_tab)
     a.dtype, a.B, a.N, a.E, a.heads = code_of(qkv), B, N, E, heads
@@ -355,8 +360,9 @@
 
 
 def attn_bwd(qkv, cos_tab, o, lse, d_o, dqkv, delta, B, N, E, heads, *, dsin=None, dfreqs=None, drop_mask=None, drop_rate=0.0, defer_freqs=False,
-             head_dim=None, sin_tab=None, grid_w=0, nkeep=None):
+             head_dim=None, sin_tab=None, grid_w=0, nkeep=None, q_rows=0):
     a = L.AttnBwdArgs()
+    a.q_rows = int(q_rows)
     if sin_tab is not None:
         a.rope_mode, a.sin_tab, a.grid_w, a.dfreqs = L.ROPE_ROTATE, _p(sin_tab), int(grid_w), _p(dfreqs) if dfreqs is not None else None
     a.dtype, a.B, a.N, a.E, a.heads = code_of(qkv), B, N, E, heads
@@ -444,6 +450,10 @@
         return
     L.check(L.lib().lnx_layerscale_bwd(_p(g), _p(z), code_of(z), _p(gamma), _p(rowscale), rows_per_sample, _p(dz), _p(dgamma), M, Cc, _stream()),
             "lnx_layerscale_bwd")
+
+
+def zero_cols(x, ld_bytes, width_bytes, M):
+    L.check(L.lib().lnx_zero_cols(_p(x), C.c_int64(ld_bytes), C.c_int64(width_bytes), M, _stream()), "lnx_zero_cols")
 
 
 def fill_rows(vec, out, ldout, row_map, M, Cc):
```

Result: no change. 14300 images/sec (median of 6 runs) (+0.1%).
